# Suyashagarw/StreamOptima

Measured on AMD Instinct MI355X. Metric: encoded Mpixels/sec at 1080p & 4K, 1/2/4/8 GPUs; PSNR delta vs reference, higher is better.
Workload: dtype u8

## Files before the change

### include/streamoptima.h

```cpp
#ifndef STREAMOPTIMA_H
#define STREAMOPTIMA_H

#include <stddef.h>
#include <stdint.h>

#ifdef __cplusplus
extern "C" {
#endif

#define SO_OK 0
#define SO_E_INVALID (-1)
#define SO_E_UNSUPPORTED (-2)
#define SO_MAX_REF 4
#define SO_ABI_VERSION 1

int so_abi_version(void);
const char* so_last_error(void);

int so_me_full_search(const uint8_t* cur, const uint8_t* const* refs, int nref, int H,
                      int W, int bs, int sr, int32_t* out_best, int32_t* out_sub,
                      void* stream);

int so_inter_tq_recon(const uint8_t* cur, const uint8_t* const* refs, int nref, int H,
                      int W, int bs, const int32_t* best, const int32_t* sub, int qp_rd,
                      const int32_t* qp_row, int vbs, double lam, uint8_t* out_split,
                      int16_t* out_mv, int16_t* out_qtc, int32_t* out_tokens,
                      int32_t* out_mae_num, uint8_t* out_recon, int32_t* out_sse, void* stream);

size_t so_p_frame_scratch_elems(int H, int W, int bs, int vbs);

int so_encode_p_frame(const uint8_t* cur, const uint8_t* const* refs, int nref, int H,
                      int W, int bs, int sr, int qp_rd, const int32_t* qp_row, int vbs,
                      double lam, uint8_t* out_split, int16_t* out_mv, int16_t* out_qtc,
                      int32_t* out_tokens, int32_t* out_mae_num, uint8_t* out_recon,
                      int32_t* out_sse, int32_t* scratch, void* stream);

int so_encode_p_rows(const uint8_t* cur, const uint8_t* const* refs, int nref, int H, int W,
                     int bs, int sr, int by0, int by1, int qp_rd, const int32_t* qp_row,
                     int vbs, double lam, uint8_t* out_split, int16_t* out_mv,
                     int16_t* out_qtc, int32_t* out_tokens, int32_t* out_mae_num,
                     uint8_t* out_recon, int32_t* out_sse, int32_t* scratch, void* stream);

#define SO_OPT_RUN_2PASS_FUSED 1
#define SO_OPT_FASTME_SERIAL 2
#define SO_OPT_FASTME_SEGMENT 3
#define SO_OPT_FASTME_WARMUP 4
#define SO_OPT_COUNT_SAD_OPS 5
#define SO_OPT_TEST_LOSE_FLAG 6
#define SO_OPT_RUN_ZERO_SKIP 7
int so_set_option(int option, int value);
int so_get_option(int option);

#define SO_P_RUN_TIMEOUT_WORD 32
#define SO_P_RUN_FALLBACK_WORD 64
#define SO_P_RUN_SAD_OPS_WORD 66
#define SO_P_RUN_STALE_WORD 33
#define SO_P_RUN_GAP_WORD 34
#define SO_P_RUN_DIAG_WORD 96
#define SO_P_RUN_DIAG_MAGIC 0x534F0001u
size_t so_p_run_workspace_elems(int H, int W);
int so_p_run_resident_workgroups(int vbs);
int so_p_run_mode_resident_workgroups(int mode, int vbs);
int so_encode_p_run(const uint8_t* const* curs, int nframes, const uint8_t* ref0, int H, int W,
                    int bs, int sr, int qp_rd, const int32_t* qp_row, int vbs, double lam,
                    uint8_t* const* out_split,
                    int16_t* const* out_mv, int16_t* const* out_qtc, int32_t* const* out_tokens,
                    int32_t* const* out_mae_num, uint8_t* const* out_recon, int32_t* const* out_sse,
                    uint32_t* workspace, void* stream);

int so_p_run_2pass_fused(int H, int W);

int so_encode_p_run_2pass(const uint8_t* const* curs, int nframes, const uint8_t* ref0, int H, int W,
                          int bs, int sr, int qp_rd, const int32_t* qp_row, const int32_t* roi,
                          int qp_lo, int qp_hi, uint8_t* const* out_split, int16_t* const* out_mv,
                          int16_t* const* out_qtc, int32_t* const* out_tokens,
                          int32_t* const* out_mae_num, uint8_t* const* out_recon,
                          int32_t* const* out_sse, int32_t* const* out_qp_map, uint32_t* workspace,
                          void* stream);

int so_encode_p_runs(const uint8_t* const* curs, int nframes, const uint8_t* const* refs,
                     const int32_t* ref_frame, int H, int W, int bs, int sr, int qp_rd,
                     const int32_t* qp_row, int vbs, double lam, uint8_t* const* out_split,
                     int16_t* const* out_mv,
                     int16_t* const* out_qtc, int32_t* const* out_tokens, int32_t* const* out_mae_num,
                     uint8_t* const* out_recon, int32_t* const* out_sse, uint32_t* workspace,
                     void* stream);

int so_encode_p_run_stripe(const uint8_t* const* curs, int nframes, const uint8_t* ref0, int H, int W,
                           int bs, int sr, int by0, int by1, int qp_rd, const int32_t* qp_row,
                           uint8_t* const* out_split, int16_t* const* out_mv, int16_t* const* out_qtc,
                           int32_t* const* out_tokens, int32_t* const* out_mae_num,
                           uint8_t* const* out_recon, int32_t* const* out_sse, uint32_t* workspace,
                           int gbase, uint8_t* peer_up0, uint8_t* peer_dn0, long long stride,
                           const uint32_t* my_up_flags, const uint32_t* my_dn_flags,
                           uint32_t* peer_up_flags, uint32_t* peer_dn_flags, uint32_t epoch, int max_wg,
                           void* stream);

int so_stripe_halo_push(const uint8_t* plane, int H, int W, int by0, int by1, int gf, uint8_t* peer_up,
                        uint8_t* peer_dn, uint32_t* peer_up_flags, uint32_t* peer_dn_flags,
                        uint32_t epoch, void* stream);

int so_encode_p_run_fpipe2(const uint8_t* const* curs, int nframes, int H, int W, int bs, int sr,
                           int qp_rd, const int32_t* qp_row, int vbs, double lam,
                           uint8_t* const* out_split,
                           int16_t* const* out_mv, int16_t* const* out_qtc, int32_t* const* out_tokens,
                           int32_t* const* out_mae_num, uint8_t* const* out_recon,
                           int32_t* const* out_sse, uint32_t* workspace, const uint8_t* land0,
                           const uint32_t* land_flags, int slot0, uint8_t* peer_land0,
                           uint32_t* peer_flags, uint8_t* peer2_land0, uint32_t* peer2_flags,
                           const int32_t* push_to, int nslots, long long stride, uint32_t epoch,
                           int max_wg, void* stream);
int so_encode_p_run_fpipe_2pass(const uint8_t* const* curs, int nframes, int H, int W, int bs, int sr,
                                int qp_rd, const int32_t* qp_row, const int32_t* roi, int qp_lo,
                                int qp_hi, uint8_t* const* out_split, int16_t* const* out_mv,
                                int16_t* const* out_qtc, int32_t* const* out_tokens,
                                int32_t* const* out_mae_num, uint8_t* const* out_recon,
                                int32_t* const* out_sse, int32_t* const* out_qp_map, uint32_t* workspace,
                                const uint8_t* land0, const uint32_t* land_flags, int slot0,
                                uint8_t* peer_land0, uint32_t* peer_flags, uint8_t* peer2_land0,
                                uint32_t* peer2_flags, const int32_t* push_to, int nslots, long long stride,
                                uint32_t epoch, int max_wg, int p2lag, void* stream);
int so_frame_push(const uint8_t* plane, int H, int W, uint8_t* peer_plane, uint32_t* peer_flags,
                  uint32_t epoch, void* stream);

#define SO_IPC_HANDLE_BYTES 64
int so_alloc_uncached(size_t bytes, void** out);
int so_free_device(void* p);
int so_ipc_export(void* p, uint8_t* out_handle);
int so_ipc_open(const uint8_t* handle, void** out);
int so_ipc_close(void* p);
int so_copy_d2d(void* dst, const void* src, size_t bytes, void* stream);
int so_memset_d8(void* dst, int value, size_t bytes, void* stream);

size_t so_i_frame_scratch_elems(int H, int W, int bs);

int so_encode_i_frame(const uint8_t* cur, int H, int W, int bs, int sr, int qp_rd,
                      const int32_t* qp_row, int vbs, double lam, uint8_t* out_split,
                      int16_t* out_mv, int16_t* out_qtc, int32_t* out_tokens,
                      int32_t* out_mae_num, uint8_t* out_recon, int32_t* out_sse,
                      int32_t* scratch, void* stream);

int so_encode_i_rows(const uint8_t* cur, int H, int W, int bs, int sr, int by0, int by1,
                     int qp_rd, const int32_t* qp_row, int vbs, double lam, uint8_t* out_split,
                     int16_t* out_mv, int16_t* out_qtc, int32_t* out_tokens,
                     int32_t* out_mae_num, uint8_t* out_recon, int32_t* out_sse,
// ... 79 lines not shown
```

### streamoptima_amd/_lib.py

```python
from __future__ import annotations

import ctypes
import os
import threading

import torch

from .build import LIB_PATH

_lock = threading.Lock()
_lib = None

SO_OK = 0
SO_E_INVALID = -1
SO_E_UNSUPPORTED = -2
MAX_REF = 4

_vp = ctypes.c_void_p
_i = ctypes.c_int
_d = ctypes.c_double
_sz = ctypes.c_size_t

_SIGS = {
    "so_abi_version": ([], _i),
    "so_last_error": ([], ctypes.c_char_p),
    "so_me_full_search": ([_vp, _vp, _i, _i, _i, _i, _i, _vp, _vp, _vp], _i),
    "so_inter_tq_recon": ([_vp, _vp, _i, _i, _i, _i, _vp, _vp, _i, _vp, _i, _d, _vp, _vp, _vp, _vp,
                           _vp, _vp, _vp, _vp], _i),
    "so_p_frame_scratch_elems": ([_i, _i, _i, _i], _sz),
    "so_encode_p_frame": ([_vp, _vp, _i, _i, _i, _i, _i, _i, _vp, _i, _d, _vp, _vp, _vp, _vp, _vp,
                           _vp, _vp, _vp, _vp], _i),
    "so_encode_p_rows": ([_vp, _vp, _i, _i, _i, _i, _i, _i, _i, _i, _vp, _i, _d, _vp, _vp, _vp, _vp,
                          _vp, _vp, _vp, _vp, _vp], _i),
    "so_p_run_workspace_elems": ([_i, _i], _sz),
    "so_p_run_resident_workgroups": ([_i], _i),
    "so_p_run_mode_resident_workgroups": ([_i, _i], _i),
    "so_p_run_2pass_fused": ([_i, _i], _i),
    "so_encode_p_run": ([_vp, _i, _vp, _i, _i, _i, _i, _i, _vp, _i, _d, _vp, _vp, _vp, _vp, _vp, _vp, _vp, _vp, _vp],
                        _i),
    "so_encode_p_run_2pass": ([_vp, _i, _vp, _i, _i, _i, _i, _i, _vp, _vp, _i, _i, _vp, _vp, _vp, _vp, _vp, _vp, _vp,
                               _vp, _vp, _vp], _i),
    "so_encode_p_runs": ([_vp, _i, _vp, _vp, _i, _i, _i, _i, _i, _vp, _i, _d, _vp, _vp, _vp, _vp, _vp, _vp, _vp, _vp,
                          _vp], _i),
    "so_i_frame_scratch_elems": ([_i, _i, _i], _sz),
    "so_encode_i_frame": ([_vp, _i, _i, _i, _i, _i, _vp, _i, _d, _vp, _vp, _vp, _vp, _vp, _vp, _vp,
                           _vp, _vp], _i),
    "so_encode_i_rows": ([_vp, _i, _i, _i, _i, _i, _i, _i, _vp, _i, _d, _vp, _vp, _vp, _vp, _vp, _vp,
                          _vp, _vp, _vp], _i),
    "so_inter_recon": ([_vp, _i, _i, _i, _i, _i, _vp, _vp, _vp, _vp, _vp, _vp], _i),
    "so_intra_recon": ([_i, _i, _i, _i, _vp, _vp, _vp, _vp, _vp, _vp, _vp], _i),
    "so_sse_u8": ([_vp, _vp, ctypes.c_int64, _vp, _vp], _i),
    "so_block_xform": ([_vp, _i, _i, _i, _i, _vp, _vp, _vp, _vp], _i),
    "so_encode_p_run_stripe": ([_vp, _i, _vp, _i, _i, _i, _i, _i, _i, _i, _vp, _vp, _vp, _vp, _vp, _vp, _vp, _vp, _vp,
                                _i, _vp, _vp, ctypes.c_longlong, _vp, _vp, _vp, _vp, ctypes.c_uint32, _i, _vp], _i),
    "so_stripe_halo_push": ([_vp, _i, _i, _i, _i, _i, _vp, _vp, _vp, _vp, ctypes.c_uint32, _vp], _i),
    "so_alloc_uncached": ([_sz, ctypes.POINTER(ctypes.c_void_p)], _i),
    "so_free_device": ([_vp], _i),
    "so_ipc_export": ([_vp, _vp], _i),
    "so_ipc_open": ([_vp, ctypes.POINTER(ctypes.c_void_p)], _i),
    "so_ipc_close": ([_vp], _i),
    "so_copy_d2d": ([_vp, _vp, _sz, _vp], _i),
    "so_memset_d8": ([_vp, _i, _sz, _vp], _i),
    "so_pack_bound": ([_i, _i], _sz),
    "so_sum_i32_rows": ([_vp, _i, _i, _vp, _vp], _i),
    "so_unpack_frames": ([_i, _vp, _vp, _vp, _i, _i, _vp, _vp, _vp, _vp, _vp], _i),
    "so_encode_p_run_fpipe2": ([_vp, _i, _i, _i, _i, _i, _i, _vp, _i, _d,
                                _vp, _vp, _vp, _vp, _vp, _vp, _vp, _vp,
                                _vp, _vp, _i, _vp, _vp, _vp, _vp, _vp, _i,
                                ctypes.c_longlong, ctypes.c_uint32, _i, _vp], _i),
    "so_encode_p_run_fpipe_2pass": ([_vp, _i, _i, _i, _i, _i, _i, _vp, _vp, _i, _i,
                                     _vp, _vp, _vp, _vp, _vp, _vp, _vp, _vp, _vp,
                                     _vp, _vp, _i, _vp, _vp, _vp, _vp, _vp, _i,
                                     ctypes.c_longlong, ctypes.c_uint32, _i, _i, _vp], _i),
    "so_frame_push": ([_vp, _i, _i, _vp, _vp, ctypes.c_uint32, _vp], _i),
    "so_pack_frames": ([_i, _vp, _vp, _vp, _vp, _i, _i, _vp, _vp, ctypes.c_ulonglong, _vp], _i),
    "so_pack_frames_ex": ([_i, _vp, _vp, _vp, _vp, _i, _i, _vp, _vp, ctypes.c_ulonglong, _vp, _vp], _i),
    "so_fme_plane_stride": ([_i, _i], _sz),
    "so_fme_workspace_bytes": ([_i, _i, _i], _sz),
    "so_fme_planes": ([_vp, _i, _i, _i, _vp, _vp], _i),
    "so_me_search_ex": ([_vp, _vp, _i, _i, _i, _i, _i, _i, _i, _i, _vp, _vp, _vp, _vp], _i),
    "so_encode_p_rows_ex": ([_vp, _vp, _i, _i, _i, _i, _i, _i, _i, _i, _vp, _vp, _i, _d, _i, _i, _i, _vp, _i,
                             _vp, _vp, _vp, _vp, _vp, _vp, _vp, _vp, _vp], _i),
    "so_inter_recon_ex": ([_vp, _i, _i, _i, _i, _i, _vp, _vp, _i, _i, _vp, _vp, _vp, _vp, _vp, _vp], _i),
    "so_encode_i_rows_ex": ([_vp, _i, _i, _i, _i, _i, _i, _i, _vp, _vp, _i, _d, _vp, _vp, _vp, _vp, _vp, _vp,
                             _vp, _vp, _vp], _i),
    "so_intra_recon_ex": ([_i, _i, _i, _i, _vp, _vp, _vp, _vp, _vp, _vp, _vp, _vp], _i),
    "so_qp_map": ([_vp, _i, _i, _i, _i, _i, _i, _vp, _vp, _i, _i, _vp, _vp], _i),
    "so_set_option": ([_i, _i], _i),
    "so_get_option": ([_i], _i),
}

ME_FULL, ME_FAST, ME_FAST_PAR = 0, 1, 2
REUSE_ME = 1
TOKENS_ONLY = 2
OPT_RUN_2PASS_FUSED, OPT_FASTME_SERIAL, OPT_FASTME_SEGMENT, OPT_FASTME_WARMUP, OPT_COUNT_SAD_OPS = 1, 2, 3, 4, 5
OPT_RUN_ZERO_SKIP = 7
OPT_TEST_LOSE_FLAG = 6

EXPORTED = tuple(_SIGS)


class HipPathError(RuntimeError):
    """Raised when the gfx950 library is unavailable or a kernel call fails."""


def load(path: str | None = None):
    global _lib
    with _lock:
        if _lib is not None:
            return _lib
        p = path or os.environ.get("SO_LIB_PATH") or LIB_PATH
        if not os.path.exists(p):
            raise HipPathError(
                f"{p} is missing: build it with `python -m streamoptima_amd.build` (hipcc, gfx950). "
                "There is no CPU fallback for the encode path.")
        lib = ctypes.CDLL(p)
        for name, (args, res) in _SIGS.items():
            if p != LIB_PATH and not hasattr(lib, name):
                continue
            fn = getattr(lib, name)
            fn.argtypes = args
            fn.restype = res
        if lib.so_abi_version() != 1:
            raise HipPathError("libstreamoptima_hip.so ABI mismatch")
        _lib = lib
        return lib


def check(rc: int, what: str) -> None:
    if rc != SO_OK:
        msg = load().so_last_error().decode(errors="replace")
        if rc == SO_E_INVALID:
            raise ValueError(f"{what}: {msg}")
        if rc == SO_E_UNSUPPORTED:
            raise NotImplementedError(f"{what}: {msg}")
        raise HipPathError(f"{what}: HIP error {rc}: {msg}")


def set_option(opt: int, value: int) -> int:
    lib = load()
    old = lib.so_get_option(opt)
    check(lib.so_set_option(opt, int(value)), "so_set_option")
    return old


class option:

    def __init__(self, opt: int, value: int):
        self.opt, self.value, self.old = opt, value, None

    def __enter__(self):
        self.old = set_option(self.opt, self.value)
        return self

    def __exit__(self, *exc):
        set_option(self.opt, self.old)
        return False


def ptr(t) -> int | None:
    return None if t is None else t.data_ptr()


def ref_array(refs) -> ctypes.Array:
    arr = (ctypes.c_void_p * len(refs))(*[r.data_ptr() for r in refs])
    return arr


def stream_handle(device=None) -> int:
    return torch.cuda.current_stream(device).cuda_stream
```

### streamoptima_amd/csrc/so_block.h

```cpp
#pragma once
#include "so_common.h"
#include "so_dct.h"

namespace so {

SO_DEV void wave_sync() {
    __builtin_amdgcn_fence(__ATOMIC_RELEASE, "wavefront");
    __builtin_amdgcn_wave_barrier();
    __builtin_amdgcn_fence(__ATOMIC_ACQUIRE, "wavefront");
}

SO_DEV int scan_index(int n, int i, int j) {
    const int k = i + j;
    const int before = (k < n) ? (k * (k + 1)) / 2 : n * n - ((2 * n - 1 - k) * (2 * n - k)) / 2;
    const int first_i = (k < n) ? 0 : k - n + 1;
    return before + (i - first_i);
}

template <int G>
SO_DEV int group_sum(int v) {
#pragma unroll
    for (int m = G / 2; m >= 1; m >>= 1) v += __shfl_xor(v, m, 64);
    return v;
}
// ... 54 lines not shown
    const uint8_t* p = f + (size_t)y * W + x;
    if constexpr (NB == 16) {
        uint4 v = *reinterpret_cast<const uint4*>(p);
        uint32_t w[4] = {v.x, v.y, v.z, v.w};
#pragma unroll
        for (int k = 0; k < 16; ++k) out[k] = (w[k >> 2] >> (8 * (k & 3))) & 255;
    } else {
        uint2 v = *reinterpret_cast<const uint2*>(p);
        uint32_t w[2] = {v.x, v.y};
#pragma unroll
        for (int k = 0; k < 8; ++k) out[k] = (w[k >> 2] >> (8 * (k & 3))) & 255;
    }
}

template <int NB>
SO_DEV void store_row_u8(uint8_t* __restrict__ f, int W, int x, int y, const int* v) {
    uint32_t w[NB / 4];
#pragma unroll
    for (int k = 0; k < NB / 4; ++k)
        w[k] = (uint32_t)(v[4 * k] & 255) | ((uint32_t)(v[4 * k + 1] & 255) << 8) |
               ((uint32_t)(v[4 * k + 2] & 255) << 16) | ((uint32_t)(v[4 * k + 3] & 255) << 24);
    uint8_t* p = f + (size_t)y * W + x;
    if constexpr (NB == 16) *reinterpret_cast<uint4*>(p) = make_uint4(w[0], w[1], w[2], w[3]);
    else *reinterpret_cast<uint2*>(p) = make_uint2(w[0], w[1]);
}

template <int NB>
SO_DEV void store_row_i16(int16_t* __restrict__ p, const int* v) {
    uint32_t w[NB / 2];
#pragma unroll
    for (int k = 0; k < NB / 2; ++k) w[k] = (uint32_t)(uint16_t)v[2 * k] | ((uint32_t)(uint16_t)v[2 * k + 1] << 16);
    if constexpr (NB == 16) {
        reinterpret_cast<uint4*>(p)[0] = make_uint4(w[0], w[1], w[2], w[3]);
        reinterpret_cast<uint4*>(p)[1] = make_uint4(w[4], w[5], w[6], w[7]);
    } else {
        reinterpret_cast<uint4*>(p)[0] = make_uint4(w[0], w[1], w[2], w[3]);
    }
}

template <int NB>
SO_DEV void load_row_i16(const int16_t* __restrict__ p, int* v) {
    uint32_t w[NB / 2];
    if constexpr (NB == 16) {
        uint4 a = reinterpret_cast<const uint4*>(p)[0], b = reinterpret_cast<const uint4*>(p)[1];
        w[0] = a.x; w[1] = a.y; w[2] = a.z; w[3] = a.w; w[4] = b.x; w[5] = b.y; w[6] = b.z; w[7] = b.w;
    } else {
        uint4 a = reinterpret_cast<const uint4*>(p)[0];
        w[0] = a.x; w[1] = a.y; w[2] = a.z; w[3] = a.w;
    }
#pragma unroll
    for (int k = 0; k < NB / 2; ++k) {
        v[2 * k] = (int)(int16_t)(w[k] & 0xFFFF);
        v[2 * k + 1] = (int)(int16_t)(w[k] >> 16);
    }
}

template <int N, bool INVERSE, class T, class TWt = typename dct::Rfft<N>::TW>
SO_DEV void xform2d_rows(double* lds, int l, const T* in_row, double* out_row, const TWt& tw = TWt{}) {
    constexpr int P = N + 1;
    double v[N];
    if constexpr (N == 16 && __is_same(T, int)) {
        int* const li = reinterpret_cast<int*>(lds);
#pragma unroll
        for (int c = 0; c < N; ++c) li[l * P + c] = in_row[c];
        wave_sync();
        int x[N];
#pragma unroll
        for (int r = 0; r < N; ++r) x[r] = li[r * P + l];
        wave_sync();
        if constexpr (INVERSE) dct::dct3_16_i(x, v, tw); else dct::dct2_16_i(x, v, tw);
    } else {
#pragma unroll
        for (int c = 0; c < N; ++c) lds[l * P + c] = (double)in_row[c];
        wave_sync();
#pragma unroll
        for (int r = 0; r < N; ++r) v[r] = lds[r * P + l];
        if constexpr (INVERSE) dct::dct3<N>(v, tw); else dct::dct2<N>(v, tw);
    }
#pragma unroll
    for (int r = 0; r < N; ++r) lds[r * P + l] = v[r];
    wave_sync();
#pragma unroll
    for (int c = 0; c < N; ++c) v[c] = lds[l * P + c];
    if constexpr (INVERSE) dct::dct3<N>(v, tw); else dct::dct2<N>(v, tw);
#pragma unroll
    for (int c = 0; c < N; ++c) out_row[c] = v[c];
    wave_sync();
}

template <class TWt>
SO_DEV void xform2d_fwd_i_half(double* lds, int l, const int* in_row, double* out_row, const TWt& tw) {
    constexpr int N = 16, PI = N + 1, P = 9;
    const int hl = l >> 3, cl = l & 7;
    double v[N];
    {
        int* const li = reinterpret_cast<int*>(lds);
#pragma unroll
        for (int c = 0; c < N; ++c) li[l * PI + c] = in_row[c];
        wave_sync();
        int x[N];
#pragma unroll
        for (int r = 0; r < N; ++r) x[r] = li[r * PI + l];
        wave_sync();
        dct::dct2_16_i(x, v, tw);
    }
#pragma unroll
    for (int h = 0; h < 2; ++h) {
        if (hl == h) {
#pragma unroll
            for (int r = 0; r < N; ++r) lds[r * P + cl] = v[r];
        }
        wave_sync();
#pragma unroll
        for (int c = 0; c < 8; ++c) out_row[8 * h + c] = lds[l * P + c];
        wave_sync();
    }
    dct::dct2<N>(out_row, tw);
}

template <bool INVERSE, class T>
SO_DEV void xform2d_rows_half(double* lds, int l, const T* in_row, double* out_row) {
    constexpr int N = 16, P = 9;
    const int hl = l >> 3, cl = l & 7;
    double v[N];
#pragma unroll
    for (int h = 0; h < 2; ++h) {
#pragma unroll
        for (int c = 0; c < 8; ++c) lds[l * P + c] = (double)in_row[8 * h + c];
        wave_sync();
        if (hl == h) {
#pragma unroll
            for (int r = 0; r < N; ++r) v[r] = lds[r * P + cl];
        }
        wave_sync();
    }
    if constexpr (INVERSE) dct::dct3<N>(v); else dct::dct2<N>(v);
#pragma unroll
    for (int h = 0; h < 2; ++h) {
        if (hl == h) {
#pragma unroll
            for (int r = 0; r < N; ++r) lds[r * P + cl] = v[r];
        }
        wave_sync();
#pragma unroll
        for (int c = 0; c < 8; ++c) out_row[8 * h + c] = lds[l * P + c];
        wave_sync();
    }
    if constexpr (INVERSE) dct::dct3<N>(out_row); else dct::dct2<N>(out_row);
}

template <bool INVERSE, class T, class TWt = dct::TW8>
SO_DEV void xform2d_sub(double* lds, int l, const T (&in)[2][8], double (&out)[2][8], const TWt& tw = TWt{}) {
    const int j = l >> 2, r0 = l & 3;
    double* s = lds + j * 72;
    if constexpr (__is_same(T, int)) {
        int* const si = reinterpret_cast<int*>(s);
#pragma unroll
        for (int h = 0; h < 2; ++h)
#pragma unroll
            for (int c = 0; c < 8; ++c) si[(r0 + 4 * h) * 9 + c] = in[h][c];
        wave_sync();
        int x[2][8];
#pragma unroll
        for (int h = 0; h < 2; ++h)
#pragma unroll
            for (int r = 0; r < 8; ++r) x[h][r] = si[r * 9 + r0 + 4 * h];
// ... 179 lines not shown
```

### streamoptima_amd/csrc/so_capi.hip

```cpp
#include <stdarg.h>
#include <stdio.h>
#include <stdlib.h>
#include <string.h>

#include <atomic>
#include <vector>

#include <hip/hip_ext.h>

#include "so_common.h"
#include "so_run.h"

namespace so {

static thread_local char g_err[512] = "";

void set_error(const char* fmt, ...) {
    va_list ap;
    va_start(ap, fmt);
    vsnprintf(g_err, sizeof(g_err), fmt, ap);
    va_end(ap);
}

static std::atomic<int> g_opt[8] = {0, 1, 0, 32, 32, 0, 0, 0};

int option(int id) {
    return (id > 0 && id < 8) ? g_opt[id].load(std::memory_order_relaxed) : 0;
}

int me_launch(const uint8_t* cur, const RefSet& refs, int nref, int H, int W, int bs, int sr, int by0, int by1,
              int32_t* out_best, int32_t* out_sub, hipStream_t st);
int me_generic_launch(const uint8_t* cur, const RefSet& refs, const uint8_t* planes, size_t pstride, int nref, int H,
                      int W, int bs, int sr, int by0, int by1, int32_t* out_best, int32_t* out_sub, hipStream_t st);
int me_fme_launch(const uint8_t* cur, const uint8_t* planes, size_t pstride, int nref, int H, int W, int by0, int by1,
                  int32_t* out_best, int32_t* out_sub, hipStream_t st);
int fme_planes_launch(const uint8_t* ref, int H, int W, int wrap, uint8_t* out, size_t pstride, hipStream_t st);
int me_fastpred_launch(const uint8_t* cur, const uint8_t* const* ptrs, int nptr, int nref, int H, int W, int bs,
                       int fme, int by0, int by1, int serial, int32_t* out_best, int32_t* out_sub, int32_t* seg_ws,
                       hipStream_t st);
constexpr size_t kFastSegWords = 2 * 4096 * 6;
int p_tile_launch(const uint8_t* cur, const RefSet& refs, int H, int W, int by0, int by1, int qp_rd,
                  const int32_t* qp_row, const int32_t* qp_map, int32_t* out_best, uint8_t* out_split,
                  int16_t* out_mv, int16_t* out_qtc, int32_t* out_tokens, int32_t* out_mae, uint8_t* out_recon,
                  int32_t* out_sse, hipStream_t st, bool tokens_only = false, const int16_t* prev_mv = nullptr);

struct PackFrame {
    const uint8_t* split;
    const int16_t* mv;
    const int16_t* qtc;
    uint32_t* offs;
    uint8_t* out;
    int frame_type;
};
size_t pack_block_bound(int bs);
struct UnpackFrame {
    const uint8_t* in;
    const uint32_t* offs;
    uint8_t* split;
    int16_t* mv;
    int16_t* qtc;
    int frame_type;
};
int unpack_frames_launch(const UnpackFrame* frames, int nframes, int nb, int bs, int32_t* err, hipStream_t st);
int pack_frames_launch(const PackFrame* frames, int nframes, int nb, int bs, unsigned long long cap, uint32_t* totals,
                       hipStream_t st);
int stripe_halo_push_launch(const uint8_t* plane, int W, int by0, int by1, uint8_t* up, uint8_t* dn,
                            uint32_t* up_flags, uint32_t* dn_flags, int gf, uint32_t epoch, hipStream_t st);
int frame_push_launch(const uint8_t* plane, int H, int W, uint8_t* dst, uint32_t* flags, uint32_t epoch,
                      hipStream_t st);

#ifdef SO_AB
extern "C" int so_debug_ab_build(void) { return 1; }
#endif

static bool use_fused(int bs, int sr, int vbs, int nref) {
    if (bs != 16 || sr != 16 || vbs || nref != 1) return false;
#ifdef SO_AB
    const char* f = getenv("SO_FUSED");
    if (f && strcmp(f, "0") == 0) return false;
    const char* impl = getenv("SO_ME_IMPL");
    return impl == nullptr || impl[0] == 0;
#else
    return true;
#endif
}

int inter_tq_launch(const uint8_t* cur, const RefSet& refs, const uint8_t* planes, size_t pstride, int H, int W,
                    int bs, int by0, int by1, const int32_t* best, const int32_t* sub, int qp_rd, const int32_t* qp_row,
                    const int32_t* qp_map, int vbs, double lam, uint8_t* out_split, int16_t* out_mv, int16_t* out_qtc, int32_t* out_tokens,
                    int32_t* out_mae, uint8_t* out_recon, int32_t* out_sse, hipStream_t st);
int inter_tq_2pass_launch(const uint8_t* cur, const RefSet& refs, int H, int W, const int32_t* best, const int32_t* t1,
                          int qp_rd, const int32_t* qp_row, const int32_t* roi, int qp_lo, int qp_hi,
                          int32_t* out_qpmap, uint8_t* out_split, int16_t* out_mv, int16_t* out_qtc,
                          int32_t* out_tokens, int32_t* out_mae, uint8_t* out_recon, int32_t* out_sse,
                          hipStream_t st);
int inter_recon_launch(const RefSet& refs, const uint8_t* planes, size_t pstride, int H, int W, int bs, int qp,
                       const int32_t* qp_row, const int32_t* qp_map, const uint8_t* split, const int16_t* mv, const int16_t* qtc,
                       uint8_t* out_recon, hipStream_t st);
int intra_encode_launch(const uint8_t* cur, int H, int W, int bs, int sr, int by0, int by1, int qp_rd,
                        const int32_t* qp_row, const int32_t* qp_map, int vbs, double lam, uint8_t* out_split, int16_t* out_mv,
                        int16_t* out_qtc, int32_t* out_tokens, int32_t* out_mae, uint8_t* out_recon,
                        int32_t* out_sse, uint8_t* idres, hipStream_t st);
int intra_recon_launch(int H, int W, int bs, int sr, int qp, const int32_t* qp_row, const int32_t* qp_map,
                       const uint8_t* split,
                       const int16_t* mv, const int16_t* qtc, uint8_t* out_recon, uint8_t* idres,
                       hipStream_t st);

static int check_vbs(const char* fn, int vbs, double lam) {
    if (vbs != 0 && vbs != 1) {
        set_error("%s: vbs must be 0 or 1", fn);
// ... 110 lines not shown
    for (int m = 32; m >= 1; m >>= 1) acc += __shfl_xor(acc, m, 64);
    if ((threadIdx.x & 63) == 0) part[threadIdx.x >> 6] = acc;
    __syncthreads();
    if (threadIdx.x == 0) {
        long long t = 0;
#pragma unroll
        for (int w = 0; w < kSumThreads / 64; ++w) t += part[w];
        out[blockIdx.x] = t;
    }
}

__global__ void __launch_bounds__(256) sse_kernel(const uint8_t* __restrict__ a, const uint8_t* __restrict__ b,
                                                  int64_t n, unsigned long long* __restrict__ out) {
    __shared__ unsigned long long part[4];
    unsigned long long acc = 0;
    const int64_t n16 = n / 16;
    const int64_t stride = (int64_t)gridDim.x * blockDim.x;
    for (int64_t i = (int64_t)blockIdx.x * blockDim.x + threadIdx.x; i < n16; i += stride) {
        const uint4 va = reinterpret_cast<const uint4*>(a)[i];
        const uint4 vb = reinterpret_cast<const uint4*>(b)[i];
        const uint32_t wa[4] = {va.x, va.y, va.z, va.w}, wb[4] = {vb.x, vb.y, vb.z, vb.w};
        uint32_t s = 0;
#pragma unroll
        for (int k = 0; k < 4; ++k)
#pragma unroll
            for (int e = 0; e < 4; ++e) {
                const int d = (int)((wa[k] >> (8 * e)) & 255) - (int)((wb[k] >> (8 * e)) & 255);
                s += (uint32_t)(d * d);
            }
        acc += s;
    }
    if (blockIdx.x == 0 && threadIdx.x == 0)
        for (int64_t i = n16 * 16; i < n; ++i) {
            const int d = (int)a[i] - (int)b[i];
            acc += (unsigned long long)(d * d);
        }
#pragma unroll
    for (int m = 32; m >= 1; m >>= 1) acc += __shfl_xor(acc, m, 64);
    if ((threadIdx.x & 63) == 0) part[threadIdx.x >> 6] = acc;
    __syncthreads();
    if (threadIdx.x == 0) atomicAdd(out, part[0] + part[1] + part[2] + part[3]);
}

__global__ void __launch_bounds__(256)
qp_map_kernel(const int32_t* __restrict__ tokens, int nbx, int by0, int qp_rd, const int32_t* __restrict__ qp_row,
              const int32_t* __restrict__ roi, int qp_lo, int qp_hi, int32_t* __restrict__ out) {
    __shared__ long long part[4];
    const int by = by0 + blockIdx.x;
    const int32_t* t = tokens ? tokens + (size_t)blockIdx.x * nbx : nullptr;
    long long m = 0;
    if (t) {
        for (int bx = threadIdx.x; bx < nbx; bx += blockDim.x) m += t[bx];
#pragma unroll
        for (int s = 32; s >= 1; s >>= 1) m += __shfl_xor(m, s, 64);
        if ((threadIdx.x & 63) == 0) part[threadIdx.x >> 6] = m;
        __syncthreads();
        m = part[0] + part[1] + part[2] + part[3];
    }
    const int base = qp_row ? qp_row[by] : qp_rd;
    for (int bx = threadIdx.x; bx < nbx; bx += blockDim.x) {
        int d = 0;
        if (t) {
            const long long tn = (long long)t[bx] * nbx;
            d = (tn >= 2 * m) + (tn >= 4 * m) - (2 * tn < m) - (4 * tn < m);
        }
        int q = base + d + (roi ? roi[(size_t)by * nbx + bx] : 0);
        q = q < qp_lo ? qp_lo : (q > qp_hi ? qp_hi : q);
        out[(size_t)by * nbx + bx] = q;
    }
}

}

using namespace so;

extern "C" {

int so_abi_version(void) { return SO_ABI_VERSION; }

int so_set_option(int opt, int value) {
    const bool ok = (opt == SO_OPT_RUN_2PASS_FUSED || opt == SO_OPT_FASTME_SERIAL || opt == SO_OPT_COUNT_SAD_OPS ||
                     opt == SO_OPT_RUN_ZERO_SKIP)
                        ? (value == 0 || value == 1)
                    : opt == SO_OPT_FASTME_SEGMENT                               ? value >= 1
                    : opt == SO_OPT_FASTME_WARMUP || opt == SO_OPT_TEST_LOSE_FLAG ? value >= 0
                                                                                 : false;
    if (!ok) {
        set_error("so_set_option: option %d value %d is unknown or out of range", opt, value);
        return SO_E_INVALID;
    }
    g_opt[opt].store(value, std::memory_order_relaxed);
    return SO_OK;
}

int so_get_option(int opt) { return option(opt); }

const char* so_last_error(void) { return g_err; }

int so_me_full_search(const uint8_t* cur, const uint8_t* const* refs, int nref, int H, int W, int bs,
                      int sr, int32_t* out_best, int32_t* out_sub, void* stream) {
    const char* fn = "so_me_full_search";
    SO_TRY(check_geom(fn, H, W, bs, out_sub != nullptr));
    SO_TRY(check_sr(fn, sr));
    SO_NEED(cur, fn);
    SO_NEED(out_best, fn);
    RefSet rs;
    SO_TRY(make_refs(fn, refs, nref, &rs));
    return me_launch(cur, rs, nref, H, W, bs, sr, 0, H / bs, out_best, out_sub, (hipStream_t)stream);
}

int so_inter_tq_recon(const uint8_t* cur, const uint8_t* const* refs, int nref, int H, int W, int bs,
                      const int32_t* best, const int32_t* sub, int qp_rd, const int32_t* qp_row, int vbs,
                      double lam, uint8_t* out_split, int16_t* out_mv, int16_t* out_qtc, int32_t* out_tokens,
                      int32_t* out_mae_num, uint8_t* out_recon, int32_t* out_sse, void* stream) {
    const char* fn = "so_inter_tq_recon";
    SO_TRY(check_geom(fn, H, W, bs, vbs));
    SO_TRY(check_qp(fn, qp_rd));
    SO_NEED(cur, fn); SO_NEED(best, fn); SO_NEED(out_split, fn); SO_NEED(out_mv, fn);
    SO_NEED(out_qtc, fn); SO_NEED(out_tokens, fn); SO_NEED(out_mae_num, fn); SO_NEED(out_recon, fn);
    if (vbs) SO_NEED(sub, fn);
    RefSet rs;
    SO_TRY(make_refs(fn, refs, nref, &rs));
    for (int i = 0; i < nref; ++i)
        if (refs[i] == out_recon) {
            set_error("%s: out_recon aliases refs[%d]", fn, i);
            return SO_E_INVALID;
        }
    return inter_tq_launch(cur, rs, nullptr, 0, H, W, bs, 0, H / bs, best, vbs ? sub : nullptr, qp_rd, qp_row, nullptr, vbs, lam,
                           out_split, out_mv, out_qtc, out_tokens, out_mae_num, out_recon, out_sse,
                           (hipStream_t)stream);
}

size_t so_p_frame_scratch_elems(int H, int W, int bs, int vbs) {
    if (bs <= 0) return 0;
    const size_t nb = (size_t)(W / bs) * (size_t)(H / bs);
    return nb * 4 + (vbs ? nb * 16 : 0) + kFastSegWords;
}

int so_encode_p_rows(const uint8_t* cur, const uint8_t* const* refs, int nref, int H, int W, int bs, int sr,
                     int by0, int by1, int qp_rd, const int32_t* qp_row, int vbs, double lam, uint8_t* out_split,
                     int16_t* out_mv, int16_t* out_qtc, int32_t* out_tokens, int32_t* out_mae_num,
                     uint8_t* out_recon, int32_t* out_sse, int32_t* scratch, void* stream) {
    const char* fn = "so_encode_p_rows";
    SO_TRY(check_geom(fn, H, W, bs, vbs));
    SO_TRY(check_sr(fn, sr));
    SO_TRY(check_qp(fn, qp_rd));
    SO_TRY(check_rows(fn, H, bs, by0, by1));
    SO_NEED(cur, fn); SO_NEED(scratch, fn); SO_NEED(out_split, fn); SO_NEED(out_mv, fn);
    SO_NEED(out_qtc, fn); SO_NEED(out_tokens, fn); SO_NEED(out_mae_num, fn); SO_NEED(out_recon, fn);
    RefSet rs;
    SO_TRY(make_refs(fn, refs, nref, &rs));
    for (int i = 0; i < nref; ++i)
        if (refs[i] == out_recon) {
            set_error("%s: out_recon aliases refs[%d]", fn, i);
            return SO_E_INVALID;
        }
    const size_t nbs = (size_t)(W / bs) * (size_t)(by1 - by0);
    int32_t* best = scratch;
    int32_t* sub = vbs ? scratch + nbs * 4 : nullptr;
    hipStream_t st = (hipStream_t)stream;
    if (use_fused(bs, sr, vbs, nref))
        return p_tile_launch(cur, rs, H, W, by0, by1, qp_rd, qp_row, nullptr, best, out_split, out_mv, out_qtc,
                             out_tokens, out_mae_num, out_recon, out_sse, st);
    SO_TRY(me_launch(cur, rs, nref, H, W, bs, sr, by0, by1, best, sub, st));
    return inter_tq_launch(cur, rs, nullptr, 0, H, W, bs, by0, by1, best, sub, qp_rd, qp_row, nullptr, vbs, lam, out_split,
                           out_mv, out_qtc, out_tokens, out_mae_num, out_recon, out_sse, st);
}

int so_encode_p_frame(const uint8_t* cur, const uint8_t* const* refs, int nref, int H, int W, int bs, int sr,
                      int qp_rd, const int32_t* qp_row, int vbs, double lam, uint8_t* out_split,
                      int16_t* out_mv, int16_t* out_qtc, int32_t* out_tokens, int32_t* out_mae_num,
                      uint8_t* out_recon, int32_t* out_sse, int32_t* scratch, void* stream) {
    if (bs <= 0) {
        set_error("so_encode_p_frame: block_size %d", bs);
        return SO_E_UNSUPPORTED;
    }
    return so_encode_p_rows(cur, refs, nref, H, W, bs, sr, 0, H / bs, qp_rd, qp_row, vbs, lam, out_split, out_mv,
                            out_qtc, out_tokens, out_mae_num, out_recon, out_sse, scratch, stream);
}

size_t so_p_run_workspace_elems(int H, int W) {
    if (H <= 0 || W <= 0) return 0;
    return p_run_workspace_words(H, W);
}

int so_p_run_resident_workgroups(int vbs) {
    const int n = p_run_capacity(vbs ? 1 : 0);
    if (n <= 0) {
        set_error("so_p_run_resident_workgroups: device query failed");
        return SO_E_INVALID;
    }
    return n;
}

int so_p_run_2pass_fused(int H, int W) {
    return H > 0 && W > 0 && option(SO_OPT_RUN_2PASS_FUSED) == 1 && p_run_2pass_fused_ok(H, W) ? 1 : 0;
}

int so_p_run_mode_resident_workgroups(int mode, int vbs) {
    if (mode < 0 || mode > 4 || (vbs && mode != 0 && mode != 2)) {
        set_error("so_p_run_mode_resident_workgroups: mode %d%s", mode, vbs ? " with vbs (modes 0, 2)" : " (0..4)");
        return SO_E_INVALID;
    }
    const int n = p_run_capacity(vbs ? 1 : 0, mode);
    if (n <= 0) {
        set_error("so_p_run_mode_resident_workgroups: device query failed");
        return SO_E_INVALID;
    }
    return n;
}

int so_encode_p_run(const uint8_t* const* curs, int nframes, const uint8_t* ref0, int H, int W, int bs, int sr,
                    int qp_rd, const int32_t* qp_row, int vbs, double lam, uint8_t* const* out_split,
                    int16_t* const* out_mv, int16_t* const* out_qtc, int32_t* const* out_tokens,
                    int32_t* const* out_mae_num, uint8_t* const* out_recon, int32_t* const* out_sse,
                    uint32_t* workspace, void* stream) {
    const char* fn = "so_encode_p_run";
    SO_TRY(check_geom(fn, H, W, bs, vbs));
    SO_TRY(check_vbs(fn, vbs, lam));
    SO_TRY(check_sr(fn, sr));
    SO_TRY(check_qp(fn, qp_rd));
    if (bs != 16 || sr != 16 || W % 128 != 0) {
        set_error("%s: covers bs 16 / sr 16 / W %% 128 == 0 (call so_encode_p_frame per frame)", fn);
        return SO_E_UNSUPPORTED;
    }
    if (nframes <= 0) return SO_OK;
    SO_NEED(curs, fn); SO_NEED(ref0, fn); SO_NEED(out_split, fn); SO_NEED(out_mv, fn); SO_NEED(out_qtc, fn);
    SO_NEED(out_tokens, fn); SO_NEED(out_mae_num, fn); SO_NEED(out_recon, fn); SO_NEED(workspace, fn);
    std::vector<PFrameOut> outs((size_t)nframes);
    for (int i = 0; i < nframes; ++i) {
        SO_NEED(curs[i], fn); SO_NEED(out_split[i], fn); SO_NEED(out_mv[i], fn); SO_NEED(out_qtc[i], fn);
        SO_NEED(out_tokens[i], fn); SO_NEED(out_mae_num[i], fn); SO_NEED(out_recon[i], fn);
        for (int j = -1; j < i; ++j)
            if (out_recon[i] == (j < 0 ? ref0 : out_recon[j])) {
                set_error("%s: out_recon[%d] aliases ref0 or another frame's reconstruction", fn, i);
                return SO_E_INVALID;
            }
        outs[i] = PFrameOut{out_split[i], out_mv[i], out_qtc[i], out_tokens[i], out_mae_num[i], out_recon[i],
                            out_sse ? out_sse[i] : nullptr};
    }
    return p_run_launch(curs, nframes, ref0, H, W, qp_rd, qp_row, vbs, lam, outs.data(), workspace,
                        (hipStream_t)stream);
}

int so_encode_p_runs(const uint8_t* const* curs, int nframes, const uint8_t* const* refs, const int32_t* ref_frame,
                     int H, int W, int bs, int sr, int qp_rd, const int32_t* qp_row, int vbs, double lam,
                     uint8_t* const* out_split, int16_t* const* out_mv, int16_t* const* out_qtc,
                     int32_t* const* out_tokens, int32_t* const* out_mae_num, uint8_t* const* out_recon,
                     int32_t* const* out_sse, uint32_t* workspace, void* stream) {
    const char* fn = "so_encode_p_runs";
    SO_TRY(check_geom(fn, H, W, bs, vbs));
    SO_TRY(check_vbs(fn, vbs, lam));
    SO_TRY(check_sr(fn, sr));
    SO_TRY(check_qp(fn, qp_rd));
    if (bs != 16 || sr != 16 || W % 128 != 0) {
        set_error("%s: covers bs 16 / sr 16 / W %% 128 == 0 (call so_encode_p_frame per frame)", fn);
        return SO_E_UNSUPPORTED;
    }
    if (nframes <= 0) return SO_OK;
    SO_NEED(curs, fn); SO_NEED(refs, fn); SO_NEED(ref_frame, fn); SO_NEED(out_split, fn); SO_NEED(out_mv, fn);
    SO_NEED(out_qtc, fn); SO_NEED(out_tokens, fn); SO_NEED(out_mae_num, fn); SO_NEED(out_recon, fn);
    SO_NEED(workspace, fn);
    std::vector<PFrameOut> outs((size_t)nframes);
    std::vector<int> deps((size_t)nframes);
    int conc = 0;
    for (int i = 0; i < nframes; ++i) {
        SO_NEED(curs[i], fn); SO_NEED(out_split[i], fn); SO_NEED(out_mv[i], fn); SO_NEED(out_qtc[i], fn);
        SO_NEED(out_tokens[i], fn); SO_NEED(out_mae_num[i], fn); SO_NEED(out_recon[i], fn);
        const int d = ref_frame[i];
        if (d >= i || d < -1) {
            set_error("%s: ref_frame[%d] = %d (must be -1 or an earlier frame of the list)", fn, i, d);
            return SO_E_INVALID;
// ... 679 lines not shown
```

### streamoptima_amd/csrc/so_me.hip

```cpp
#include <stdlib.h>
#include <string.h>

#include <cstring>
#include <map>
#include <mutex>
#include <utility>

#include "so_block.h"
#include "so_common.h"
#include "so_dpp.h"
#include "so_run.h"

namespace so {

SO_DEV uint64_t me_key(uint32_t sad, uint32_t l1, uint32_t ref, uint32_t scan) {
    return ((uint64_t)sad << 32) | ((uint64_t)l1 << 24) | ((uint64_t)ref << 16) | (uint64_t)scan;
}
constexpr uint64_t kNoKey = ~0ull;
constexpr uint32_t kDenseSadOps = 1152u * 256u;
#define SO_OPS_ADD(p, v) do { if (L.count_ops) atomicAdd((p), (v)); } while (0)

SO_DEV void decode_key(uint64_t k, int sr, int32_t* out) {
    if (k == kNoKey) {
        out[0] = 0; out[1] = 0; out[2] = 0; out[3] = -1;
        return;
    }
    const int d = 2 * sr + 1;
    const int scan = (int)(k & 0xFFFF);
    out[0] = scan / d - sr;
    out[1] = scan % d - sr;
    out[2] = (int)((k >> 16) & 0xFF);
    out[3] = (int)(k >> 32);
}

template <int BS, bool SUB>
struct MeWGeo {
    static constexpr int SR = 16, D = 33, NT = 17;
    static constexpr int TBX = 128 / BS;
    static constexpr int TPY = SUB ? 32 : 64;
    static constexpr int TBY = TPY / BS;
    static constexpr int TPX = 128;
    static constexpr int WR = TPY + 2 * SR;
    static constexpr int RPD = (TPX + 2 * SR) / 4 + 1;
    static constexpr int CSTRIDE = WR * RPD + 8;
    static constexpr int NBLK = TBX * TBY;
    static constexpr int NW = SUB ? 8 : 16, NTHREADS = NW * 64;
};

typedef const __attribute__((address_space(4))) uint32_t* const_u32p;
typedef const volatile __attribute__((address_space(3))) uint32_t* lds_vu32p;

template <int NR, int NDW>
SO_DEV void load_cur_sgpr(const uint8_t* __restrict__ cur, int W, int x, int y, uint32_t (&cr)[NR][NDW]) {
#pragma unroll
    for (int r = 0; r < NR; ++r) {
        const_u32p p = (const_u32p)(cur + (size_t)(y + r) * W + x);
#pragma unroll
        for (int k = 0; k < NDW; ++k) cr[r][k] = p[k];
    }
}


template <int WR, int RPD, int CS, int NT>
SO_DEV void stage_window(uint32_t* win, const uint8_t* __restrict__ ref, int H, int W, int gx0, int gy0, int tid) {
    constexpr int N = WR * RPD, IT = (N + NT - 1) / NT;
    uint32_t a[IT], b[IT];
#pragma unroll
    for (int k = 0; k < IT; ++k) {
        const int i = tid + k * NT;
        const int wr = i / RPD, m = i - wr * RPD;
        const int gy = gy0 + wr, gx = gx0 + 4 * m;
        a[k] = 0;
        b[k] = 0;
        if (i < N && gy >= 0 && gy < H) {
            const uint8_t* rp = ref + (size_t)gy * W;
            if (gx >= 0 && gx + 4 <= W) a[k] = *reinterpret_cast<const uint32_t*>(rp + gx);
            if (gx + 4 >= 0 && gx + 8 <= W) b[k] = *reinterpret_cast<const uint32_t*>(rp + gx + 4);
        }
    }
#pragma unroll
    for (int k = 0; k < IT; ++k) {
        const int i = tid + k * NT;
        if (i < N) {
            uint32_t* d = win + i;
            d[0] = a[k];
            d[CS] = __builtin_amdgcn_alignbyte(b[k], a[k], 1);
            d[2 * CS] = __builtin_amdgcn_alignbyte(b[k], a[k], 2);
            d[3 * CS] = __builtin_amdgcn_alignbyte(b[k], a[k], 3);
// ... 329 lines not shown
        else decode_key(keys[i], 2 * SR, out_sub + (b * 4 + ((i - G::NBLK) & 3)) * 4);
    }
}

__global__ void __launch_bounds__(256)
fme_planes_kernel(const uint8_t* __restrict__ ref, int H, int W, int wrap, uint8_t* __restrict__ out, size_t pstride) {
    const int q = blockIdx.x * blockDim.x + threadIdx.x;
    const int qpr = W >> 2;
    if (q >= qpr * H) return;
    const int i = q / qpr, j0 = (q - i * qpr) * 4;
    const uint8_t* r0 = ref + (size_t)i * W + j0;
    const bool down = i + 1 < H;
    const uint8_t* r1 = down ? r0 + W : r0;
    uint32_t p00 = 0, p01 = 0, p10 = 0, p11 = 0;
    const uint32_t w0 = *reinterpret_cast<const uint32_t*>(r0), w1 = *reinterpret_cast<const uint32_t*>(r1);
    const bool right = j0 + 4 < W;
    const int e0 = right ? r0[4] : 0, e1 = right ? r1[4] : 0;
#pragma unroll
    for (int k = 0; k < 4; ++k) {
        const int a = (w0 >> (8 * k)) & 255, c = (w1 >> (8 * k)) & 255;
        const bool rk = j0 + k + 1 < W;
        const int a2 = k < 3 ? (int)((w0 >> (8 * k + 8)) & 255) : e0;
        const int c2 = k < 3 ? (int)((w1 >> (8 * k + 8)) & 255) : e1;
        int h0 = a + a2, h1 = c + c2;
        if (wrap) { h0 &= 255; h1 &= 255; }
        p00 |= (uint32_t)a << (8 * k);
        if (rk) p01 |= (uint32_t)((h0 + 1) >> 1) << (8 * k);
        if (down) p10 |= (uint32_t)((a + c + 1) >> 1) << (8 * k);
        if (down && rk) p11 |= (uint32_t)((h0 + h1 + 3) >> 2) << (8 * k);
    }
    const size_t o = (size_t)i * W + j0;
    *reinterpret_cast<uint32_t*>(out + o) = p00;
    *reinterpret_cast<uint32_t*>(out + pstride + o) = p01;
    *reinterpret_cast<uint32_t*>(out + 2 * pstride + o) = p10;
    *reinterpret_cast<uint32_t*>(out + 3 * pstride + o) = p11;
}

int fme_planes_launch(const uint8_t* ref, int H, int W, int wrap, uint8_t* out, size_t pstride, hipStream_t st) {
    const int n = (W / 4) * H;
    hipLaunchKernelGGL(fme_planes_kernel, dim3((n + 255) / 256), dim3(256), 0, st, ref, H, W, wrap, out, pstride);
    return check_launch("fme_planes_kernel");
}

int me_fme_launch(const uint8_t* cur, const uint8_t* planes, size_t pstride, int nref, int H, int W, int by0, int by1,
                  int32_t* out_best, int32_t* out_sub, hipStream_t st) {
    const int nbx = W / 16, nrows = by1 - by0;
    if (nrows <= 0) return SO_OK;
    const bool sub = out_sub != nullptr;
    const int tby = (sub ? MeWGeo<16, true>::TPY : MeWGeo<16, false>::TPY) / 16;
    const dim3 grid(((nbx + 7) / 8) * ((nrows + tby - 1) / tby));
    if (sub)
        hipLaunchKernelGGL((me_fme_kernel<true>), grid, dim3(MeWGeo<16, true>::NTHREADS), 0, st, cur, planes, pstride,
                           nref, H, W, by0, by1, out_best, out_sub);
    else
        hipLaunchKernelGGL((me_fme_kernel<false>), grid, dim3(MeWGeo<16, false>::NTHREADS), 0, st, cur, planes,
                           pstride, nref, H, W, by0, by1, out_best, out_sub);
    return check_launch("me_fme_kernel");
}

#ifndef SO_SEA2_WPE
#define SO_SEA2_WPE 6
#endif
#ifndef SO_SEA_CAP
#define SO_SEA_CAP 384
#endif
#ifndef SO_SEA_CAP_VBS
#define SO_SEA_CAP_VBS 384
#endif
#ifndef SO_DENSE_THR
#define SO_DENSE_THR 8
#endif
#ifndef SO_DENSE_PROBE
#define SO_DENSE_PROBE 16
#endif
#ifndef SO_VBS_HALVES
#define SO_VBS_HALVES 0
#endif
#ifndef SO_B4_PD
#define SO_B4_PD 2
#endif
#ifndef SO_PTILE_WPE16
#define SO_PTILE_WPE16 8
#endif
template <int NW_, int TPX_ = 128>
struct Sea2GeoT {
    static constexpr int SR = 16, NT = 17;
    static constexpr int TPX = TPX_, TBX = TPX / 16, TPY = 32, TBY = 2;
    static constexpr int WR = TPY + 2 * SR;
    static constexpr int WD = (TPX + 2 * SR) / 4;
    static constexpr int RP = WD + 1;
    static constexpr int B4R = WR - 3, B4C = TPX + 2 * SR - 3, B4P = 4 * RP;
    static constexpr int TQ_BPW = TPX == 128 ? 4 : 2;
    static constexpr int B4BAND = NW_ >= 16 ? 3 : 6;
    static constexpr int B4NB = (B4R + B4BAND - 1) / B4BAND;
    static constexpr int B4RS = B4NB * B4BAND;
    static constexpr int NBLK = TBX * TBY;
    static constexpr int NW = NW_, NTHREADS = NW * 64;
    static constexpr int CAP = SO_SEA_CAP, CAPV = SO_SEA_CAP_VBS;
    static constexpr int CAPLV = SO_VBS_HALVES ? 2 * CAPV : CAPV;
    static constexpr int CAPL = CAP > CAPLV ? CAP : CAPLV;
    static constexpr int DCS = WR * RP + 8;
    static constexpr int CPD = TPX / 4 + 1;
    static_assert(WD * B4NB <= NTHREADS, "byte-sum threads");
};
using Sea2Geo = Sea2GeoT<8>;

template <int RP>
SO_DEV uint32_t win_u32(const uint32_t* win, int row, int col) {
    lds_vu32p p = (lds_vu32p)(win + row * RP + (col >> 2));
    return __builtin_amdgcn_alignbyte(p[1], p[0], (uint32_t)(col & 3));
}

#ifdef SO_STAMPS
__device__ unsigned long long* g_sea_stamps = nullptr;
__device__ unsigned long long* g_run_stamps = nullptr;
__shared__ unsigned long long* s_stamp_rec;
#define SO_SEA_STAMP(i, v) do { if (tid == 0 && s_stamp_rec) s_stamp_rec[(i)] = (v); } while (0)
#define SO_STAMP_REC_SET(p) do { if (threadIdx.x == 0) s_stamp_rec = (p); } while (0)
extern "C" int so_debug_set_sea_stamps(void* p) {
    return (int)hipMemcpyToSymbol(HIP_SYMBOL(g_sea_stamps), &p, sizeof(p));
}
extern "C" int so_debug_set_run_stamps(void* p) {
    return (int)hipMemcpyToSymbol(HIP_SYMBOL(g_run_stamps), &p, sizeof(p));
}
#else
#define SO_STAMP_REC_SET(p) do { } while (0)
#define SO_SEA_STAMP(i, v) do { } while (0)
#endif

#define SO_MARK_NAMES(X) X(loop_top) X(stage_cur) X(stage_cur_int) X(stage_cur_edge) X(cur_sums) X(wait) \
    X(poll_iter) X(stage_win) X(stage_win_int) X(stage_win_edge) X(dense_tile) X(dense_tile_block) X(byte_sums) \
    X(block_top) X(bound) X(umin) X(umin_edge) X(ballots) X(bal_row) X(dense_fallback) X(survivors) X(sur_one) X(sur_le4) X(sur_pass) \
    X(search_end) X(decode_keys) X(tq_residual) X(tq_fwd) X(tq_quant) X(tq_tokens) X(tq_qtc_store) X(tq_inv) \
    X(tq_recon) X(tq_sse_records) X(post) X(done_flag) X(task_end) X(vbs_block) X(vbs_umin) X(vbs_list_a) \
    X(vbs_pass) X(vbs_list_b) X(vbs_final) X(vbs_dense) X(vbs_fwd) X(vbs_fwd_sub) X(vbs_final_q) X(vbs_inv) \
    X(vbs_inv_split) X(vbs_inv_end) X(wait_w0) X(keys_tail) X(p1_tq) X(p1_flag) X(p2_wait) X(p2_sums) X(p2_tq) \
    X(p2_flag)
#define SO_MARK_ENUM(n) kMark_##n,
enum SoMarkId { SO_MARK_NAMES(SO_MARK_ENUM) kMarkCount };
#undef SO_MARK_ENUM
#if defined(SO_MARKS_COUNT)
__device__ unsigned* g_mark_counts = nullptr;
__shared__ unsigned s_mark_cnt[64];
extern "C" int so_debug_set_mark_counts(void* p) {
    return (int)hipMemcpyToSymbol(HIP_SYMBOL(g_mark_counts), &p, sizeof(p));
}
SO_DEV void so_mark_hit(int id) {
    uint64_t sv, m;
    uint32_t f;
    asm volatile(
        "s_mov_b64 %0, exec\n\t"
        "s_ff1_i32_b64 %2, exec\n\t"
        "s_lshl_b64 %1, 1, %2\n\t"
        "s_and_b64 exec, exec, %1\n\t"
        "ds_add_u32 %3, %4\n\t"
        "s_mov_b64 exec, %0"
        : "=&s"(sv), "=&s"(m), "=&s"(f)
        : "v"((uint32_t)(uintptr_t)&s_mark_cnt[id]), "v"(1u)
        : "memory", "scc");
}
#define SO_MARK(name) so_mark_hit(kMark_##name)
#elif defined(SO_MARKS)
#define SO_MARK(name) asm volatile(";SO_MARK " #name)
#else
#define SO_MARK(name) do { } while (0)
#endif

SO_DEV int opaque_tid() {
    int t = threadIdx.x;
    asm volatile("" : "+v"(t));
    return t;
}

struct Sea2Lds {
    uint32_t* win;
    uint32_t* b4w;
// ... 326 lines not shown
        nB = vbs_list_from_masks<NT>(mylist, mB, cbase, 32 * 33 + d2, (uint32_t)CAP);
    } else {
#pragma unroll
        for (int t = 0; t <= NT; ++t) {
            const bool pass = t < NT ? (any_sub(T[t], Bt[t]) && ((amask >> t) & 1u) == 0u)
                                     : (ok2 && any_sub(l2T, l2B) && !(lb2 <= qU));
            const uint64_t bal = __builtin_amdgcn_ballot_w64(pass);
            if (bal) {
                const uint32_t pos = nB + lane_prefix(bal);
                if (pass && pos < (uint32_t)CAP) mylist[pos] = (uint16_t)(t < NT ? cbase + t : 32 * 33 + d2);
                nB += (uint32_t)__builtin_popcountll(bal);
            }
        }
    }
    if (nB > (uint32_t)CAP) return false;
    if (lane == 0) SO_OPS_ADD(&L.st[2], 16u * ((nB + 15) / 16) * 256u);
    __builtin_amdgcn_fence(__ATOMIC_RELEASE, "wavefront");
    __builtin_amdgcn_wave_barrier();
    __builtin_amdgcn_fence(__ATOMIC_ACQUIRE, "wavefront");
    vbs_eval_list<G>(L, mylist, nB, cs, bxl, byl, lane, bestB, best0, best1);
    SO_MARK(vbs_final);
    const uint64_t kb = wave_min_u64_dpp(bestB);
    const auto widen = [](uint32_t k) {
        return ((uint64_t)(k >> 17) << 32) | ((uint64_t)((k >> 11) & 63u) << 24) | (uint64_t)(k & 2047u);
    };
    const uint64_t kTL = widen(wave_min_u32(top ? best0 : ~0u)), kTR = widen(wave_min_u32(top ? best1 : ~0u));
    const uint64_t kBL = widen(wave_min_u32(top ? ~0u : best0)), kBR = widen(wave_min_u32(top ? ~0u : best1));
    if (lane == 0) {
        unsigned long long* const ks = L.keys;
        if (kb < ks[u]) ks[u] = kb;
        unsigned long long* const sk = ks + G::NBLK + 4 * u;
        if (kTL < sk[0]) sk[0] = kTL;
        if (kTR < sk[1]) sk[1] = kTR;
        if (kBL < sk[2]) sk[2] = kBL;
        if (kBR < sk[3]) sk[3] = kBR;
    }
    return true;
}

template <class G, class Pre = NoPre, bool VBS = false, int LISTS = 0>
SO_DEV void sea2_tile(const Sea2Lds& L, int tile, const uint8_t* __restrict__ cur, const RefSet& refs, int nref,
                      int H, int W, int by0, int by1, int probe, const Pre& pre = Pre(),
                      const int* dense_flag = nullptr, const int16_t* prev_mv = nullptr) {
    constexpr int SR = G::SR, TBX = G::TBX, TBY = G::TBY, RP = G::RP, NT = G::NT;
    constexpr int B4P = G::B4P, CAP = G::CAP, CP = G::TPX;
#ifdef SO_NO_MV_HINT
    prev_mv = nullptr;
#endif
    uint32_t* const win = L.win;
    uint32_t* const b4w = L.b4w;
    uint8_t* const b4 = reinterpret_cast<uint8_t*>(b4w);
    uint32_t* const curt = L.curt;
    uint32_t* const a4 = L.a4;
    uint16_t* const list = L.list;
    unsigned long long* const keys = L.keys;

    const int nbx = W / 16;
    const int tiles_x = (nbx + TBX - 1) / TBX;
    const int tx = tile % tiles_x, ty = tile / tiles_x;
    const bool ballot_lists = LISTS == 2 || (LISTS == 0 && SO_VBS_BALLOT_LATENCY && VBS &&
                                             tiles_x * ((H / 16 + TBY - 1) / TBY) < (int)gridDim.x);
    const int bx0 = tx * TBX, byt0 = by0 + ty * TBY;
    const int x0 = bx0 * 16, y0 = byt0 * 16;
    const int tid = opaque_tid();
    const int wave = __builtin_amdgcn_readfirstlane(tid >> 6);
    uint32_t& st_fb = L.st[0];
    if (tid == 0) st_fb = 0;
    uint32_t& st_ops = L.st[2];
    if (tid == 0) {
        uint32_t ops0 = L.count_ops ? G::NBLK * 16 * 4 * 4 : 0u;
        asm volatile("" : "+v"(ops0));
        st_ops = ops0;
    }
#ifdef SO_STAMPS
    uint32_t& st_sur = L.st[1];
    if (tid == 0) st_sur = 0;
    SO_SEA_STAMP(0, __builtin_amdgcn_s_memrealtime());
    SO_SEA_STAMP(1, __builtin_amdgcn_s_memtime());
#endif

    SO_MARK(stage_cur);
    for (int i = tid; i < G::NBLK * (VBS ? 5 : 1); i += G::NTHREADS) keys[i] = kNoKey;
    constexpr int WTPR = G::NTHREADS / G::WR, WNPT = (RP + WTPR - 1) / WTPR;
    static_assert(G::NTHREADS % G::WR == 0, "window staging");
    const int wwr = tid / WTPR, wc0 = tid - wwr * WTPR;
    const bool win_int = x0 - SR >= 0 && x0 - SR + 4 * RP <= W && y0 - SR >= 0 && y0 - SR + G::WR <= H;
    if (x0 + CP <= W && y0 + G::TPY <= H) {
        constexpr int TPR = G::NTHREADS / G::TPY, NPT = (CP / 4) / TPR;
        static_assert(G::NTHREADS % G::TPY == 0 && (CP / 4) % TPR == 0, "current-tile staging");
        SO_MARK(stage_cur_int);
        const int rr = tid / TPR, c0 = tid - rr * TPR;
        const uint32_t* src = reinterpret_cast<const uint32_t*>(cur + (size_t)(y0 + rr) * W + x0) + c0;
        uint32_t v[NPT];
#pragma unroll
        for (int k = 0; k < NPT; ++k) v[k] = src[k * TPR];
#pragma unroll
        for (int k = 0; k < NPT; ++k) curt[rr * G::CPD + c0 + k * TPR] = v[k];
    } else {
        SO_MARK(stage_cur_edge);
        constexpr int N = G::TPY * CP / 4, IT = (N + G::NTHREADS - 1) / G::NTHREADS;
        uint32_t v[IT];
#pragma unroll
        for (int k = 0; k < IT; ++k) {
            const int i = tid + k * G::NTHREADS;
            const int rr = i / (CP / 4), m = i - rr * (CP / 4);
            const int gy = y0 + rr, gx = x0 + 4 * m;
            v[k] = 0;
            if (i < N && gy < H && gx + 4 <= W) v[k] = *reinterpret_cast<const uint32_t*>(cur + (size_t)gy * W + gx);
        }
#pragma unroll
        for (int k = 0; k < IT; ++k)
            if (tid + k * G::NTHREADS < N) {
                const int i = tid + k * G::NTHREADS, rr = i / (CP / 4);
                curt[i + rr] = v[k];
            }
    }
    __syncthreads();
    SO_MARK(cur_sums);
    for (int i = tid; i < G::NBLK * 16; i += G::NTHREADS) {
        const int blk = i >> 4, j = (i >> 2) & 3, ii = i & 3;
        const int rr = (blk / TBX) * 16 + 4 * j, m = (blk % TBX) * 4 + ii;
        uint32_t sum = 0;
#pragma unroll
        for (int q = 0; q < 4; ++q) sum = __builtin_amdgcn_sad_u8(curt[(rr + q) * G::CPD + m], 0u, sum);
        reinterpret_cast<uint8_t*>(a4)[i] = (uint8_t)(sum >> 4);
    }
    uint32_t* const grab = L.lcount;
    const auto next_block = [&](int u) -> int {
#ifdef SO_SEA_STATIC
        return u + G::NW;
#else
        (void)u;
        uint32_t nx = 0;
        if ((tid & 63) == 0) nx = __hip_atomic_fetch_add(grab, 1u, __ATOMIC_RELAXED, __HIP_MEMORY_SCOPE_WORKGROUP);
        return (int)__builtin_amdgcn_readfirstlane(nx);
#endif
    };
    for (int r = 0; r < nref; ++r) {
        const uint8_t* ref = refs.p[r];
        SO_MARK(wait);
        if (r == 0) pre();
        SO_MARK(stage_win);
        if (tid == 0) *grab = (uint32_t)G::NW;
        __syncthreads();
        if (r == 0) SO_SEA_STAMP(2, __builtin_amdgcn_s_memtime());
        if (win_int) {
            SO_MARK(stage_win_int);
            uint32_t wv0[WNPT];
            const uint32_t* src = reinterpret_cast<const uint32_t*>(ref + (size_t)(y0 - SR + wwr) * W + (x0 - SR)) + wc0;
#pragma unroll
            for (int k = 0; k < WNPT; ++k)
                if (wc0 + k * WTPR < RP) wv0[k] = src[k * WTPR];
#pragma unroll
            for (int k = 0; k < WNPT; ++k)
                if (wc0 + k * WTPR < RP) win[wwr * RP + wc0 + k * WTPR] = wv0[k];
        } else {
            SO_MARK(stage_win_edge);
            constexpr int N = G::WR * RP, IT = (N + G::NTHREADS - 1) / G::NTHREADS;
            uint32_t v[IT];
#pragma unroll
            for (int k = 0; k < IT; ++k) {
                const int i = tid + k * G::NTHREADS;
                const int wr = i / RP, m = i - wr * RP;
                const int gy = y0 - SR + wr, gx = x0 - SR + 4 * m;
                v[k] = 0;
                if (i < N && gy >= 0 && gy < H && gx >= 0 && gx + 4 <= W)
                    v[k] = *reinterpret_cast<const uint32_t*>(ref + (size_t)gy * W + gx);
            }
#pragma unroll
            for (int k = 0; k < IT; ++k)
                if (tid + k * G::NTHREADS < N) win[tid + k * G::NTHREADS] = v[k];
        }
        __syncthreads();
        if (r == 0) SO_SEA_STAMP(3, __builtin_amdgcn_s_memtime());
        if (probe == 5) continue;
        if (dense_flag && __builtin_amdgcn_readfirstlane(*dense_flag)) {
            SO_MARK(dense_tile);
            const int c1 = L.dense4;
            if (c1 != 0) {
                uint32_t* const cp = win + c1;
                for (int i = tid; i < G::WR * RP; i += G::NTHREADS) {
                    const uint32_t a = win[i], b = win[i + 1];
                    cp[i] = __builtin_amdgcn_alignbyte(b, a, 1);
                    cp[G::DCS + i] = __builtin_amdgcn_alignbyte(b, a, 2);
                    cp[2 * G::DCS + i] = __builtin_amdgcn_alignbyte(b, a, 3);
                }
                __syncthreads();
            }
#pragma unroll 1
            for (int u = wave; u < G::NBLK; u = next_block(u)) {
                SO_MARK(dense_tile_block);
                const int bxl = u % TBX, byl = u / TBX;
                if (bx0 + bxl >= nbx || byt0 + byl >= by1) continue;
                const int x = x0 + bxl * 16, y = y0 + byl * 16;
                if (c1 != 0) {
                    if (VBS && x != 0 && y != 0)
                        wave_dense_block<16, true, RP, G::DCS>(win, keys, G::NBLK, cur, W, H, x, y, bxl, byl, u, tid, r,
                                                               FmePhase{0, 0}, c1);
                    else
                        wave_dense_block<16, false, RP, G::DCS>(win, keys, G::NBLK, cur, W, H, x, y, bxl, byl, u, tid,
                                                                r, FmePhase{0, 0}, c1);
                } else if (VBS && x != 0 && y != 0)
                    wave_dense_block<16, true, RP, 0, false, true>(win, keys, G::NBLK, cur, W, H, x, y, bxl, byl, u,
                                                                   tid, r);
                else
                    wave_dense_block<16, false, RP, 0, false, true>(win, keys, G::NBLK, cur, W, H, x, y, bxl, byl, u,
                                                                    tid, r);
                if ((tid & 63) == 0) {
                    atomicAdd(&st_fb, 1u);
                    SO_OPS_ADD(&st_ops, kDenseSadOps);
                }
            }
            continue;
        }
        SO_MARK(byte_sums);
        if (tid == 0) SO_OPS_ADD(&st_ops, (uint32_t)(G::WD * G::B4NB * (G::B4BAND + 3) * 4 * 4));
        if (tid < G::WD * G::B4NB) {
            const int m = tid % G::WD, band = tid / G::WD;
            const int r0 = band * G::B4BAND;
            constexpr int NR = G::B4BAND + 3;
            uint32_t h[NR][2];
            lds_vu32p p = (lds_vu32p)(win + r0 * RP + m);
#pragma unroll
            for (int i = 0; i < NR; ++i) {
                const uint32_t w0 = p[i * RP], w1 = p[i * RP + 1];
                h[i][0] = __builtin_amdgcn_sad_hi_u8(__builtin_amdgcn_alignbyte(w1, w0, 2), 0u,
                                                     __builtin_amdgcn_sad_u8(w0, 0u, 0u));
                h[i][1] = __builtin_amdgcn_sad_hi_u8(__builtin_amdgcn_alignbyte(w1, w0, 3), 0u,
                                                     __builtin_amdgcn_sad_u8(__builtin_amdgcn_alignbyte(w1, w0, 1), 0u, 0u));
            }
            typedef unsigned short so_v2u16 __attribute__((ext_vector_type(2)));
            uint8_t* const ob = b4 + r0 * B4P + m;
#pragma unroll
            for (int i = 0; i < G::B4BAND; ++i)
#pragma unroll
                for (int j = 0; j < 2; ++j) {
                    const uint32_t sum = h[i][j] + h[i + 1][j] + h[i + 2][j] + h[i + 3][j];
                    const uint32_t q = __builtin_bit_cast(uint32_t, __builtin_bit_cast(so_v2u16, sum) >> (so_v2u16){4, 4});
// ... 208 lines not shown
                for (int rr = 0; rr < 4; ++rr)
#pragma unroll
                    for (int k = 0; k < 4; ++k) cr[rr][k] = curt[crow0 + (4 * q + rr) * G::CPD + k];
#pragma unroll 1
                for (uint32_t s0 = 0; s0 < nsur; s0 += 16) {
                    SO_MARK(sur_pass);
                    const bool act = s0 + (uint32_t)sidx < nsur;
                    const int cand = act ? (int)mylist[s0 + sidx] : cs;
                    const int dxi = cand / 33, di = cand - dxi * 33;
                    const int col = bxl * 16 + dxi;
                    const uint32_t sh = (uint32_t)(col & 3);
                    int wo = (byl * 16 + di + 4 * q) * RP + (col >> 2);
                    asm volatile("" : "+v"(wo));
                    uint32_t sad = 0;
#pragma unroll
                    for (int rr = 0; rr < 4; ++rr) {
                        lds_vu32p p = (lds_vu32p)(win + wo + rr * RP);
                        const uint32_t q0 = p[0], q1 = p[1], q2 = p[2], q3 = p[3], q4 = p[4];
                        sad = __builtin_amdgcn_sad_u8(cr[rr][0], __builtin_amdgcn_alignbyte(q1, q0, sh), sad);
                        sad = __builtin_amdgcn_sad_u8(cr[rr][1], __builtin_amdgcn_alignbyte(q2, q1, sh), sad);
                        sad = __builtin_amdgcn_sad_u8(cr[rr][2], __builtin_amdgcn_alignbyte(q3, q2, sh), sad);
                        sad = __builtin_amdgcn_sad_u8(cr[rr][3], __builtin_amdgcn_alignbyte(q4, q3, sh), sad);
                    }
                    sad = quad_sum_u32(sad);
                    const int dx = dxi - 16, dy = di - 16;
                    const uint64_t key = me_key(sad, (uint32_t)((dx < 0 ? -dx : dx) + (dy < 0 ? -dy : dy)),
                                                (uint32_t)r, (uint32_t)cand);
                    best = (act && key < best) ? key : best;
                }
            }
            best = wave_min_u64_dpp(best);
            if (lane == 0 && best < keys[u]) keys[u] = best;
        }
    }
    SO_MARK(search_end);
    __syncthreads();
}

__global__ void __launch_bounds__(Sea2Geo::NTHREADS) __attribute__((amdgpu_waves_per_eu(SO_SEA2_WPE)))
me_sea2_kernel(const uint8_t* __restrict__ cur, RefSet refs, int nref, int H, int W, int by0, int by1,
               int32_t* __restrict__ out_best, int probe) {
    using G = Sea2Geo;
    constexpr int SR = G::SR, TBX = G::TBX, TBY = G::TBY, RP = G::RP, B4P = G::B4P;
    __shared__ uint32_t win[G::WR * RP + 4];
    __shared__ uint32_t b4w[(G::B4RS * B4P + 4) / 4];
    __shared__ uint32_t curt[G::TPY * G::CPD];
    __shared__ uint32_t a4[G::NBLK * 4];
    __shared__ uint16_t list[G::NW * G::CAPL];
    __shared__ uint32_t lcount[G::NW];
    __shared__ unsigned long long keys[G::NBLK];
    __shared__ uint32_t st[3];
    const Sea2Lds L{win, b4w, curt, a4, list, lcount, keys, st};
    SO_STAMP_REC_SET(g_sea_stamps ? g_sea_stamps + (size_t)blockIdx.x * 12 : nullptr);
    sea2_tile<Sea2Geo>(L, blockIdx.x, cur, refs, nref, H, W, by0, by1, probe);

    const int tid = threadIdx.x;
    const int nbx = W / 16;
    const int tiles_x = (nbx + TBX - 1) / TBX;
    const int bx0 = (blockIdx.x % tiles_x) * TBX, byt0 = by0 + (blockIdx.x / tiles_x) * TBY;
    SO_SEA_STAMP(5, __builtin_amdgcn_s_memtime());
    for (int i = tid; i < G::NBLK; i += G::NTHREADS) {
        const int gbx = bx0 + i % TBX, gby = byt0 + i / TBX;
        if (gbx >= nbx || gby >= by1) continue;
        decode_key(keys[i], SR, out_best + ((size_t)(gby - by0) * nbx + gbx) * 4);
    }
#ifdef SO_STAMPS
    if (tid == 0) {
        uint32_t hw, xcc;
        asm volatile("s_getreg_b32 %0, hwreg(HW_REG_HW_ID)" : "=s"(hw));
        asm volatile("s_getreg_b32 %0, hwreg(HW_REG_XCC_ID)" : "=s"(xcc));
        SO_SEA_STAMP(6, __builtin_amdgcn_s_memtime());
        SO_SEA_STAMP(7, __builtin_amdgcn_s_memrealtime());
        SO_SEA_STAMP(8, ((unsigned long long)xcc << 32) | hw);
        SO_SEA_STAMP(9, ((unsigned long long)st[0] << 32) | st[1]);
    }
#endif
}

constexpr int kTqScratch = 16 * 17;
#ifndef SO_PTILE_TOK_HALF
#define SO_PTILE_TOK_HALF 1
#endif
constexpr int kTqScratchHalf = 16 * 9;
#ifndef SO_FWD_MFMA
#define SO_FWD_MFMA 0
#endif
template <class G, bool HALFTQ = false>
struct PTileGeo {
    static constexpr int B4 = (G::B4RS * G::B4P + 4) / 4;
    static constexpr int LIST = G::NW * G::CAPL / 2;
    static constexpr int TQD = G::NBLK * (HALFTQ ? kTqScratchHalf : kTqScratch);
    static constexpr int U64 = ((B4 + LIST + 1) / 2 > TQD) ? (B4 + LIST + 1) / 2 : TQD;
};
constexpr int kTqScratchVbs = 288;
template <class G>
struct PTileGeoVbs {
    static constexpr int TQD = G::NBLK * kTqScratchVbs;
    static constexpr int U64 = ((PTileGeo<G>::B4 + PTileGeo<G>::LIST + 1) / 2 > TQD)
                                   ? (PTileGeo<G>::B4 + PTileGeo<G>::LIST + 1) / 2 : TQD;
};

template <int RP>
SO_DEV void win_row16(const uint32_t* win, int row, int col, uint32_t (&w)[4]) {
    lds_vu32p p = (lds_vu32p)(win + row * RP + (col >> 2));
    const uint32_t sh = (uint32_t)(col & 3);
    const uint32_t q0 = p[0], q1 = p[1], q2 = p[2], q3 = p[3], q4 = p[4];
    w[0] = __builtin_amdgcn_alignbyte(q1, q0, sh);
    w[1] = __builtin_amdgcn_alignbyte(q2, q1, sh);
    w[2] = __builtin_amdgcn_alignbyte(q3, q2, sh);
    w[3] = __builtin_amdgcn_alignbyte(q4, q3, sh);
}

typedef uint32_t so_v4u __attribute__((ext_vector_type(4)));

struct MeRec {
    uint16_t v[4];
    SO_DEV int operator[](int k) const { return k < 3 ? (int)(int16_t)v[k] : (v[3] == 0xFFFFu ? -1 : (int)v[3]); }
    SO_DEV void set(const int32_t (&r)[4]) {
#pragma unroll
        for (int k = 0; k < 4; ++k) v[k] = (uint16_t)r[k];
    }
};

template <class G, bool VBS = false, bool HALFTQ = false>
struct PTileLds {
    static constexpr int NU = G::NBLK * (VBS ? 5 : 1);
    uint32_t win[G::WR * G::RP + 4];
    uint32_t curt[G::TPY * G::CPD];
    uint32_t a4[G::NBLK * 4];
    uint32_t lcount[G::NW];
    unsigned long long keys[NU];
    uint32_t st[3];
    MeRec mer[NU];
    int32_t msum[G::TBY];
    uint32_t fwd_flags;
    alignas(16) double un[VBS ? PTileGeoVbs<G>::U64 : PTileGeo<G, HALFTQ>::U64];
    uint8_t vsp[VBS ? G::NBLK : 1];
};

struct PHalo {
    uint8_t* up;
    uint8_t* dn;
    int up_end, dn_begin;
};

#ifdef SO_TQ_TW_LITERAL
#define SO_TQ_TW() dct::TW16{}
#define SO_TQ_TW8() dct::TW8{}
#else
#define SO_TQ_TW() dct::tw16_table()
#define SO_TQ_TW8() dct::tw8_table()
#endif
template <class G, bool SC1, bool HALO = false, bool TOK = false, bool HALFTQ = false, bool ZSKIP = false>
SO_DEV void tq16_exact(PTileLds<G, false, HALFTQ>& S, int g, int l, double* scratch, int bx0, int byt0, int nbx, int by0, int by1,
                       int W, int qp_rd, const int32_t* __restrict__ qp_row, const int32_t* __restrict__ qp_map,
                       const PFrameOut& o, const PHalo& hl = PHalo{}, bool qs = false) {
    constexpr int SR = G::SR, TBX = G::TBX;
    const int bxl = g % TBX, byl = g / TBX;
    const int gbx = bx0 + bxl, gby = byt0 + byl;
    if (gbx < nbx && gby < by1) {
        const size_t b = (size_t)(gby - by0) * nbx + gbx;
        const int x = gbx * 16, y = gby * 16;
        const int qpr = qp_map ? qp_map[(size_t)gby * nbx + gbx] : (qp_row ? qp_row[gby] : qp_rd);
        const int dx = S.mer[g][0], dy = S.mer[g][1], rf = S.mer[g][2], sad = S.mer[g][3];
        const int prow = byl * 16 + SR + dy + l, pcol = bxl * 16 + SR + dx;
        const uint32_t* crow = S.curt + (byl * 16 + l) * G::CPD + bxl * 4;
        double* dl = scratch;
        constexpr double kRne = 0x1.8p52;
        int q[16];
        if (qs) {
            const so_v4u* qr = reinterpret_cast<const so_v4u*>(reinterpret_cast<const int16_t*>(dl) + l * 16);
#pragma unroll
            for (int h = 0; h < 2; ++h) {
                const so_v4u v = qr[h];
#pragma unroll
                for (int e = 0; e < 4; ++e) {
                    q[8 * h + 2 * e] = (int)(int16_t)(v[e] & 0xFFFFu);
                    q[8 * h + 2 * e + 1] = (int)v[e] >> 16;
                }
            }
        } else {
            SO_MARK(tq_residual);
            int res[16];
            {
                uint32_t pw[4];
                win_row16<G::RP>(S.win, prow, pcol, pw);
#pragma unroll
                for (int k = 0; k < 4; ++k) {
                    const uint32_t cw = crow[k];
#pragma unroll
                    for (int e = 0; e < 4; ++e)
                        res[4 * k + e] = (int)((cw >> (8 * e)) & 255) - (int)((pw[k] >> (8 * e)) & 255);
                }
            }
            double tcr[16];
            SO_MARK(tq_fwd);
            static_assert(!HALFTQ || TOK, "the half scratch carries the forward transform only");
            if constexpr (HALFTQ)
                xform2d_fwd_i_half(dl, l, res, tcr, SO_TQ_TW());
            else
                xform2d_rows<16, false>(dl, l, res, tcr, SO_TQ_TW());
            SO_MARK(tq_quant);
#pragma unroll
            for (int c = 0; c < 16; ++c)
                q[c] = (int)(uint32_t)__builtin_bit_cast(
                    uint64_t, __builtin_amdgcn_ldexp(__builtin_rint(tcr[c]), -q_exp_fast<16>(l, c, qpr)) + kRne);
        }
        SO_MARK(tq_tokens);
        const int tok = block_tokens<16>(nullptr, l, q);
        if constexpr (TOK) {
            if (l == 0) o.tokens[b] = tok;
            return;
        }
        SO_MARK(tq_qtc_store);
        store_row_i16<16>(o.qtc + b * 256 + l * 16, q);
        const auto finish = [&](const int (&rec)[16]) -> int {
            if constexpr (SC1) {
                so_v4u v;
#pragma unroll
                for (int k = 0; k < 4; ++k)
                    v[k] = (uint32_t)(rec[4 * k] & 255) | ((uint32_t)(rec[4 * k + 1] & 255) << 8) |
                           ((uint32_t)(rec[4 * k + 2] & 255) << 16) | ((uint32_t)(rec[4 * k + 3] & 255) << 24);
                uint8_t* rp = o.recon + (size_t)(y + l) * W + x;
                asm volatile("global_store_dwordx4 %0, %1, off sc1" ::"v"(rp), "v"(v) : "memory");
                if constexpr (HALO) {
                    if (hl.up && y + l < hl.up_end) {
                        uint8_t* q2 = hl.up + (size_t)(y + l) * W + x;
                        asm volatile("global_store_dwordx4 %0, %1, off sc0 sc1" ::"v"(q2), "v"(v) : "memory");
                    }
                    if (hl.dn && y + l >= hl.dn_begin) {
                        uint8_t* q2 = hl.dn + (size_t)(y + l) * W + x;
                        asm volatile("global_store_dwordx4 %0, %1, off sc0 sc1" ::"v"(q2), "v"(v) : "memory");
                    }
                }
            } else {
                store_row_u8<16>(o.recon, W, x, y + l, rec);
            }
            SO_MARK(tq_sse_records);
            int e2 = 0;
            if (o.sse) {
#pragma unroll
                for (int k = 0; k < 4; ++k) {
                    const uint32_t cw = crow[k];
#pragma unroll
                    for (int e = 0; e < 4; ++e) {
                        const int d = (int)((cw >> (8 * e)) & 255) - (rec[4 * k + e] & 255);
                        e2 += d * d;
                    }
                }
                e2 = group_sum<16>(e2);
            }
            return e2;
        };
        const auto full = [&]() -> int {
            int dq[16];
            double rd[16];
            dequant_row_int<16>(q, l, qpr, dq);
            SO_MARK(tq_inv);
            xform2d_rows<16, true>(dl, l, dq, rd, SO_TQ_TW());
            SO_MARK(tq_recon);
            int rec[16];
            {
                uint32_t pw[4];
                win_row16<G::RP>(S.win, prow, pcol, pw);
#pragma unroll
                for (int c = 0; c < 16; ++c)
                    rec[c] = (int)((pw[c >> 2] >> (8 * (c & 3))) & 255) +
                             (int)(uint32_t)__builtin_bit_cast(uint64_t, rd[c] + kRne);
            }
            return finish(rec);
        };
        int sse;
        if constexpr (ZSKIP) {
            if (__builtin_amdgcn_ballot_w64(tok != 1) == 0) {
                int rec[16];
                uint32_t pw[4];
                win_row16<G::RP>(S.win, prow, pcol, pw);
#pragma unroll
                for (int c = 0; c < 16; ++c) rec[c] = (int)((pw[c >> 2] >> (8 * (c & 3))) & 255);
                sse = finish(rec);
            } else {
                sse = full();
            }
        } else {
            sse = full();
        }
        if (l < 12) o.mv[b * 12 + l] = (int16_t)(l == 0 ? dx : l == 1 ? dy : l == 2 ? rf : 0);
        if (l == 0) {
            o.split[b] = 0;
            o.tokens[b] = tok;
            o.mae[b] = sad;
            if (o.sse) o.sse[b] = sse;
        }
    }
}

__constant__ float kDctCos32[17] = {
    0x1.6a09e6p-2f, 0x1.684b9cp-2f, 0x1.63150cp-2f, 0x1.5a730cp-2f, 0x1.4e7aeap-2f, 0x1.3f4a24p-2f,
    0x1.2d062ep-2f, 0x1.17dc14p-2f, 0x1.000000p-2f, 0x1.cb598cp-3f, 0x1.92469cp-3f, 0x1.5553e4p-3f,
    0x1.1517a8p-3f, 0x1.a4608ap-4f, 0x1.1a855ep-4f, 0x1.1be352p-5f, 0.0f};

SO_DEV float dct16_f32(int u, int r) {
    if (u == 0) return 0.25f;
    const int j = ((2 * r + 1) * u) & 63;
    const int m = j <= 32 ? j : 64 - j;
    return m <= 16 ? kDctCos32[m] : -kDctCos32[32 - m];
}

typedef float so_v4f __attribute__((ext_vector_type(4)));
constexpr float kFwdBound = 2.6e-7f;

template <class G>
SO_DEV void fwd_mfma(PTileLds<G>& S, int g, int ln, const float (&cs)[4], int bx0, int byt0, int nbx, int by1,
                     int qp_rd, const int32_t* __restrict__ qp_row, const int32_t* __restrict__ qp_map) {
    constexpr int SR = G::SR, TBX = G::TBX;
    const int bxl = g % TBX, byl = g / TBX;
    const int gbx = bx0 + bxl, gby = byt0 + byl;
    if (gbx >= nbx || gby >= by1) return;
    const int qpr = qp_map ? qp_map[(size_t)gby * nbx + gbx] : (qp_row ? qp_row[gby] : qp_rd);
    const int r = ln & 15, c4 = ln >> 4;
    const int dx = S.mer[g][0], dy = S.mer[g][1];
    const uint32_t cw = S.curt[(byl * 16 + r) * G::CPD + bxl * 4 + c4];
    const uint32_t pw = win_u32<G::RP>(S.win, byl * 16 + SR + dy + r, bxl * 16 + SR + dx + 4 * c4);
    float a[4];
    uint32_t sab = 0;
#pragma unroll
    for (int s = 0; s < 4; ++s) {
        const int d = (int)((cw >> (8 * s)) & 255) - (int)((pw >> (8 * s)) & 255);
        a[s] = (float)d;
        sab += (uint32_t)(d < 0 ? -d : d);
    }
    sab = wave_sum_u32(sab);
    so_v4f y = {0.f, 0.f, 0.f, 0.f}, z = {0.f, 0.f, 0.f, 0.f};
#pragma unroll
    for (int s = 0; s < 4; ++s) y = __builtin_amdgcn_mfma_f32_16x16x4f32(a[s], cs[s], y, 0, 0, 0);
#pragma unroll
    for (int s = 0; s < 4; ++s) z = __builtin_amdgcn_mfma_f32_16x16x4f32(cs[s], y[s], z, 0, 0, 0);
    const float delta = __builtin_fmaf((float)sab, kFwdBound, 0x1p-20f);
    bool near = qpr < 1;
    int16_t* qd = reinterpret_cast<int16_t*>(S.un + g * kTqScratch);
#pragma unroll
    for (int i = 0; i < 4; ++i) {
        const int u = 4 * c4 + i, k = q_exp_fast<16>(u, r, qpr);
        const float zi = z[i];
        const float mid = __builtin_amdgcn_ldexpf(__builtin_floorf(__builtin_amdgcn_ldexpf(zi, -k)) + 0.5f, k);
        near |= __builtin_fabsf(__builtin_fabsf(zi - mid) - 0.5f) <= delta;
        qd[u * 16 + r] = (int16_t)(int)__builtin_rintf(__builtin_amdgcn_ldexpf(__builtin_rintf(zi), -k));
    }
#ifdef SO_FWD_FORCE
    near = SO_FWD_FORCE;
#endif
    if (__builtin_amdgcn_ballot_w64(near) != 0 && ln == 0) atomicOr(&S.fwd_flags, 1u << g);
}

template <int NBLK>
SO_DEV int fwd_order(uint32_t m, int p) {
    const int nf = __builtin_popcount(m);
    uint32_t s = p < nf ? m : (~m & ((1u << NBLK) - 1u));
    for (int t = p < nf ? p : p - nf; t > 0; --t) s &= s - 1u;
    return __builtin_ctz(s);
}

template <int RP>
SO_DEV void win_row8(const uint32_t* win, int row, int col, uint32_t (&w)[2]) {
    lds_vu32p p = (lds_vu32p)(win + row * RP + (col >> 2));
    const uint32_t sh = (uint32_t)(col & 3);
    const uint32_t q0 = p[0], q1 = p[1], q2 = p[2];
    w[0] = __builtin_amdgcn_alignbyte(q1, q0, sh);
    w[1] = __builtin_amdgcn_alignbyte(q2, q1, sh);
}

template <bool SC1, bool HALO>
SO_DEV void store_rec_row(const PFrameOut& o, const PHalo& hl, int W, int x, int yy, const int* rec, int n) {
    uint8_t* rp = o.recon + (size_t)yy * W + x;
// ... 336 lines not shown
                       int by0, int by1, int qp_rd, const int32_t* __restrict__ qp_row,
                       const int32_t* __restrict__ qp_map, int32_t* __restrict__ out_best, const PFrameOut& o,
                       const Pre& pre = Pre(), const PHalo& hl = PHalo{}, double lam = 0.0,
                       const int* dense_flag = nullptr, int32_t* fb_out = nullptr, int count_ops = 0,
                       const Post& post = Post(), const int16_t* prev_mv = nullptr) {
    constexpr int SR = G::SR, TBX = G::TBX, TBY = G::TBY;
    using P = PTileGeo<G>;
    uint32_t* const b4w = reinterpret_cast<uint32_t*>(S.un);
    uint16_t* const list = reinterpret_cast<uint16_t*>(b4w + P::B4);
    constexpr int kUnDw = 2 * (VBS ? PTileGeoVbs<G>::U64 : PTileGeo<G, HALFTQ>::U64);
    int dense4 = 0;
#ifndef SO_DENSE_ONE
    if constexpr (3 * G::DCS + 32 <= kUnDw) {
        const int d = (int)((reinterpret_cast<uintptr_t>(b4w) - reinterpret_cast<uintptr_t>(S.win)) / 4);
        dense4 = d + ((8 - d) & 31);
    }
#endif
    const Sea2Lds L{S.win, b4w, S.curt, S.a4, list, S.lcount, S.keys, S.st, count_ops, dense4};
    RefSet refs{};
    refs.p[0] = ref;
#ifndef SO_PROF_PHASE
#define SO_PROF_PHASE 0
#endif
    sea2_tile<G, Pre, VBS, LISTS>(L, tile, cur, refs, 1, H, W, by0, by1, SO_PROF_PHASE == 2 ? 5 : 0, pre,
                           dense_flag, prev_mv);

    const int tid = opaque_tid();
    SO_SEA_STAMP(5, __builtin_amdgcn_s_memtime());
    const int nbx = W / 16;
    const int tiles_x = (nbx + TBX - 1) / TBX;
    const int bx0 = (tile % tiles_x) * TBX, byt0 = by0 + (tile / tiles_x) * TBY;
    for (int i = tid; i < PTileLds<G, VBS>::NU; i += G::NTHREADS) {
        SO_MARK(decode_keys);
        int32_t rec4[4];
        decode_key(S.keys[i], SR, rec4);
        S.mer[i].set(rec4);
        const int gbx = bx0 + i % TBX, gby = byt0 + i / TBX;
        if (out_best && i < G::NBLK && gbx < nbx && gby < by1) {
            int32_t* ob = out_best + ((size_t)(gby - by0) * nbx + gbx) * 4;
            ob[0] = S.mer[i][0]; ob[1] = S.mer[i][1]; ob[2] = S.mer[i][2]; ob[3] = S.mer[i][3];
        }
    }
    SO_MARK(keys_tail);
    if (fb_out != nullptr && tid == 0) store_sc1_i32(fb_out, (int)S.st[0]);
    if (tid == 0) S.fwd_flags = 0u;
    __syncthreads();
    SO_SEA_STAMP(6, __builtin_amdgcn_s_memtime());
    constexpr bool kFwdMfma = !VBS && SO_FWD_MFMA && SO_PROF_PHASE != 1;
    if constexpr (kFwdMfma) {
        const int ln = tid & 63;
        float cs[4];
#pragma unroll
        for (int s = 0; s < 4; ++s) cs[s] = dct16_f32(ln & 15, 4 * (ln >> 4) + s);
        for (int g = tid >> 6; g < G::NBLK; g += G::NW)
            fwd_mfma<G>(S, g, ln, cs, bx0, byt0, nbx, by1, qp_rd, qp_row, qp_map);
        __syncthreads();
#ifdef SO_FWD_COUNT
        if (tid == 0) S.st[2] = (uint32_t)__builtin_popcount(S.fwd_flags);
#endif
    }
    {
        const int ln = tid & 63, w = tid >> 6;
        int gq = w * G::TQ_BPW + (ln >> 4);
        bool qs = false;
        if constexpr (kFwdMfma) {
            const uint32_t m = S.fwd_flags;
            if (m != 0u && gq < G::NBLK) gq = fwd_order<G::NBLK>(m, gq);
            qs = !((m >> gq) & 1u);
        }
        if (SO_PROF_PHASE == 1 && ln < 16 * G::TQ_BPW && gq < G::NBLK) {
            const int bxl = gq % G::TBX, byl = gq / G::TBX, l = ln & 15;
            const int gbx = bx0 + bxl, gby = byt0 + byl;
            if (gbx < nbx && gby < by1) {
                const uint32_t* crow = S.curt + (byl * 16 + l) * G::CPD + bxl * 4;
                so_v4u v;
                for (int k = 0; k < 4; ++k) v[k] = crow[k];
                *reinterpret_cast<so_v4u*>(o.recon + (size_t)(gby * 16 + l) * W + gbx * 16) = v;
            }
        } else if (ln < 16 * G::TQ_BPW && gq < G::NBLK) {
            if constexpr (VBS)
                tq16_vbs_fwd<G, SC1, HALO>(S, gq, ln & 15, S.un + gq * kTqScratchVbs, bx0, byt0, nbx, by0, by1, W, qp_rd,
                                           qp_row, qp_map, lam, o);
            else
                tq16_exact<G, SC1, HALO, TOK, HALFTQ, ZSKIP>(S, gq, ln & 15, S.un + gq * (HALFTQ ? kTqScratchHalf : kTqScratch), bx0,
                                              byt0, nbx, by0, by1, W, qp_rd,
                                              qp_row, qp_map, o, hl, qs);
        }
    }
    if constexpr (VBS) {
        if (SO_PROF_PHASE != 1) {
            __syncthreads();
            const int ln = tid & 63, gq = (tid >> 6) * G::TQ_BPW + (ln >> 4);
            if (ln < 16 * G::TQ_BPW && gq < G::NBLK)
                tq16_vbs_inv<G, SC1, HALO>(S, gq, ln & 15, S.un, bx0, byt0, nbx, by0, by1, W, qp_rd,
                                           qp_row, qp_map, o, hl);
        }
    }
    SO_SEA_STAMP(7, __builtin_amdgcn_s_memtime());
    SO_MARK(post);
    post();
    if constexpr (SC1) asm volatile("s_waitcnt vmcnt(0)" ::: "memory");
    SO_SEA_STAMP(14, __builtin_amdgcn_s_memtime());
    __syncthreads();
}



template <class G>
SO_DEV void tq16_pass1(PTileLds<G>& S, int g, int l, double* scratch, int bx0, int byt0, int nbx, int by1, int qp_rd,
                       const int32_t* __restrict__ qp_row, const PFrameOut& o, int32_t* __restrict__ t1) {
    constexpr int SR = G::SR, TBX = G::TBX;
    const int bxl = g % TBX, byl = g / TBX;
    const int gbx = bx0 + bxl, gby = byt0 + byl;
    if (gbx < nbx && gby < by1) {
        const size_t b = (size_t)gby * nbx + gbx;
        const int qpr = qp_row ? qp_row[gby] : qp_rd;
        const int dx = S.mer[g][0], dy = S.mer[g][1], rf = S.mer[g][2], sad = S.mer[g][3];
        const int prow = byl * 16 + SR + dy + l, pcol = bxl * 16 + SR + dx;
        const uint32_t* crow = S.curt + (byl * 16 + l) * G::CPD + bxl * 4;
        int res[16];
        {
            uint32_t pw[4];
            win_row16<G::RP>(S.win, prow, pcol, pw);
#pragma unroll
            for (int k = 0; k < 4; ++k) {
                const uint32_t cw = crow[k];
#pragma unroll
                for (int e = 0; e < 4; ++e)
                    res[4 * k + e] = (int)((cw >> (8 * e)) & 255) - (int)((pw[k] >> (8 * e)) & 255);
            }
            const so_v4u pv{pw[0], pw[1], pw[2], pw[3]};
            uint8_t* const rp = o.recon + (size_t)(gby * 16 + l) * (nbx * 16) + gbx * 16;
            asm volatile("global_store_dwordx4 %0, %1, off sc1" ::"v"(rp), "v"(pv) : "memory");
        }
        double tcr[16];
        xform2d_rows<16, false>(scratch, l, res, tcr, SO_TQ_TW());
        constexpr double kRne = 0x1.8p52;
        int tc[16], q[16];
#pragma unroll
        for (int c = 0; c < 16; ++c) tc[c] = (int)(uint32_t)__builtin_bit_cast(uint64_t, tcr[c] + kRne);
        quant_row_int<16>(tc, l, qpr, q);
        const int tok = block_tokens<16>(nullptr, l, q);
        {
            uint32_t w[8];
#pragma unroll
            for (int k = 0; k < 8; ++k) w[k] = (uint32_t)(uint16_t)tc[2 * k] | ((uint32_t)tc[2 * k + 1] << 16);
            const so_v4u v0{w[0], w[1], w[2], w[3]}, v1{w[4], w[5], w[6], w[7]};
            int16_t* const qp_ = o.qtc + b * 256 + l * 16;
            asm volatile("global_store_dwordx4 %0, %1, off sc1" ::"v"(qp_), "v"(v0) : "memory");
            asm volatile("global_store_dwordx4 %0, %1, off offset:16 sc1" ::"v"(qp_), "v"(v1) : "memory");
        }
        if (l < 12) store_sc1_i16(o.mv + b * 12 + l, l == 0 ? dx : l == 1 ? dy : l == 2 ? rf : 0);
        if (l == 0) {
            o.split[b] = 0;
            o.mae[b] = sad;
            store_sc1_i32(t1 + b, tok);
        }
    }
}

SO_DEV void row16_any(const uint8_t* p, uint32_t (&w)[4]) {
    const uint32_t* pa = reinterpret_cast<const uint32_t*>((uintptr_t)p & ~(uintptr_t)3);
    const uint32_t sh = (uint32_t)((uintptr_t)p & 3);
    uint32_t q5[5];
#pragma unroll
    for (int k = 0; k < 5; ++k) q5[k] = pa[k];
#pragma unroll
// ... 189 lines not shown
                break;
        }
#endif
        __builtin_amdgcn_s_sleep(1);
        const uint32_t now = (uint32_t)(__builtin_amdgcn_s_memrealtime() - t0), gap = now - last;
        last = now;
        if (gap >= (uint32_t)kRunGapTicks) {
            susp += gap;
            __hip_atomic_fetch_add(&ws[kRunGapWord], one, __ATOMIC_RELAXED, __HIP_MEMORY_SCOPE_AGENT);
        }
        const uint32_t active = now - susp;
        if (!esc && active > (uint32_t)kRunEscalateTicks) {
            esc = true;
            const uint32_t v2 = (need && !sysl) ? rmw_read(c) : raw;
            const uint32_t v3 = (need && !sysl) ? __hip_atomic_load(c, __ATOMIC_RELAXED, __HIP_MEMORY_SCOPE_AGENT) : raw;
            if (__builtin_amdgcn_ballot_w64(need && !sysl && !ok && v2 == w.want && v3 != w.want) != 0)
                __hip_atomic_fetch_add(&ws[kRunStaleWord], one, __ATOMIC_RELAXED, __HIP_MEMORY_SCOPE_AGENT);
        }
        if (active > (uint32_t)w.limit) {
            __hip_atomic_fetch_add(&ws[kRunTimeoutWord], one, __ATOMIC_RELAXED, __HIP_MEMORY_SCOPE_AGENT);
            const uint32_t claim = __builtin_amdgcn_readfirstlane(
                __hip_atomic_fetch_add(&ws[kRunClaimWord], one, __ATOMIC_RELAXED, __HIP_MEMORY_SCOPE_AGENT));
            if (claim == 0u) {
                const uint32_t rv = (need && !sysl) ? rmw_read(c) : raw;
                const uint64_t bneed = __builtin_amdgcn_ballot_w64(need);
                const uint64_t bsys = __builtin_amdgcn_ballot_w64(need && sysl);
                const uint64_t brmw = __builtin_amdgcn_ballot_w64(need && !sysl && rv == w.want);
                const uint32_t other = (uint32_t)__builtin_amdgcn_ds_bpermute(((lane - 20) & 63) << 2, (int)raw);
                uint32_t hw, xcc;
                asm volatile("s_getreg_b32 %0, hwreg(HW_REG_HW_ID)" : "=s"(hw));
                asm volatile("s_getreg_b32 %0, hwreg(HW_REG_XCC_ID)" : "=s"(xcc));
                if (lane >= 20 && lane < 32)
                    __hip_atomic_store(&ws[kRunDiagWord + lane], other, __ATOMIC_RELAXED, __HIP_MEMORY_SCOPE_AGENT);
                if (lane == 0) {
                    const uint32_t rec[19] = {(uint32_t)w.task, (uint32_t)w.f, (uint32_t)w.dep, (uint32_t)w.tile, w.want,
                                              w.sys_want, (uint32_t)w.mode | (esc ? 1u << 12 : 0u), (uint32_t)bneed,
                                              (uint32_t)bsys, active, now, susp, 0u, 0xFFFFFFFFu, hw, xcc,
                                              (uint32_t)blockIdx.x, (uint32_t)gridDim.x, (uint32_t)brmw};
#pragma unroll
                    for (int i = 0; i < 19; ++i)
                        __hip_atomic_store(&ws[kRunDiagWord + 1 + i], rec[i], __ATOMIC_RELAXED, __HIP_MEMORY_SCOPE_AGENT);
                }
                const unsigned long long ta = __builtin_amdgcn_s_memrealtime();
                uint32_t arrive = 0xFFFFFFFFu;
                for (;;) {
                    const uint32_t x = sysl ? __hip_atomic_load(c, __ATOMIC_RELAXED, __HIP_MEMORY_SCOPE_SYSTEM)
                                            : (need ? rmw_read(c) : 0u);
                    const uint32_t el = (uint32_t)(__builtin_amdgcn_s_memrealtime() - ta);
                    if (__builtin_amdgcn_ballot_w64(need && x != (sysl ? w.sys_want : w.want)) == 0) {
                        arrive = el;
                        break;
                    }
                    if (el > 5000000u) break;
                    __builtin_amdgcn_s_sleep(8);
                }
                if (lane == 14)
                    __hip_atomic_store(&ws[kRunDiagWord + 14], arrive, __ATOMIC_RELAXED, __HIP_MEMORY_SCOPE_AGENT);
                if (lane == 0)
                    __hip_atomic_store(&ws[kRunDiagWord], SO_P_RUN_DIAG_MAGIC, __ATOMIC_RELAXED,
                                       __HIP_MEMORY_SCOPE_AGENT);
            }
            break;
        }
    }
    return raw;
}


SO_DEV uint32_t run_dequeue(uint32_t* ws) {
    uint32_t r;
    uint64_t sv;
    asm volatile(
        "s_mov_b64 %1, exec\n\t"
        "s_mov_b64 exec, 1\n\t"
        "global_atomic_add %0, %2, %3, off sc0\n\t"
        "s_waitcnt vmcnt(0)\n\t"
        "s_mov_b64 exec, %1"
        : "=&v"(r), "=&s"(sv)
        : "v"(ws), "v"(1u)
        : "memory");
    return r;
}

template <int NW, int MODE, bool VBS = false, bool HOOKS = false, bool UQP = false, bool ZSKIP = false>
__global__ void __launch_bounds__(NW * 64)
__attribute__((amdgpu_waves_per_eu(VBS ? SO_VBS_WPE : (NW >= 16 ? SO_PTILE_WPE16 : SO_SEA2_WPE))))
p_run_kernel(const PRunArgs a, int nframes, const uint8_t* __restrict__ ref0, int H, int W,
             int qp_rd, const int32_t* __restrict__ qp_row_arg, uint32_t* __restrict__ ws, int ws_stamp_base,
             const PRunStripe sp, double lam) {
    static_assert(!UQP || VBS, "the uniform-QP instantiation is the VBS run's");
    static_assert(!ZSKIP || (MODE == kRunSingle && !HOOKS && (!VBS || UQP)),
                  "the zero-skip / latency-lists instantiation is the one-GPU run's");
    constexpr int LISTS = VBS && MODE == kRunSingle && UQP ? (ZSKIP ? 2 : 1) : 0;
    const int32_t* __restrict__ const qp_row = UQP ? nullptr : qp_row_arg;
    using G = Sea2GeoT<NW>;
    __shared__ PTileLds<G, VBS> S;
    __shared__ int s_task;
    __shared__ int s_dense;
    const int tid = threadIdx.x;
    const int nbx = W / 16;
    constexpr bool STRIPE = MODE == kRunStripe, FPIPE = MODE == kRunFPipe || MODE == kRunFPipe2P;
    constexpr bool TWOP = MODE == kRunTwoPass || MODE == kRunFPipe2P;
    static_assert(!(VBS && (TWOP || MODE == kRunStripe)), "VBS runs: one GPU and the frame pipeline");
    static_assert(!HOOKS || MODE == kRunSingle, "test hooks: the one-GPU run only");
    const int count_ops = HOOKS ? sp.count_ops : 0;
    const int by0 = STRIPE ? sp.by0 : 0, by1 = STRIPE ? sp.by1 : H / 16;
    const int tiles_x = (nbx + G::TBX - 1) / G::TBX, ntr = (by1 - by0 + G::TBY - 1) / G::TBY;
    const int ntiles = tiles_x * ntr;
    constexpr bool MERGE2P = MODE == kRunTwoPass;
    const int lag2 = ntiles - (tiles_x + 1);
    const int per_frame = TWOP && !MERGE2P ? 2 * ntiles : ntiles;
    const int ntasks = per_frame * nframes + (MERGE2P ? lag2 : 0);
    uint32_t* const done = ws + kRunDoneBase;
    uint32_t* const tilefb = ws + kRunDoneBase + 2 * (size_t)kRunMax * ntiles + (size_t)kRunMax * nbx * (H / 16);
    const int wave = __builtin_amdgcn_readfirstlane(tid >> 6);
    const int lane = tid & 63;
    const uint32_t one = lane == 0 ? 1u : 0u;
    __shared__ uint32_t s_fbsum;
    __shared__ unsigned long long s_ops;
    if (tid == 0) {
        s_fbsum = 0;
        s_ops = 0;
    }
#ifdef SO_MARKS_COUNT
    if (tid < 64) s_mark_cnt[tid] = 0u;
#endif
    const uint32_t ep0 = __builtin_amdgcn_readfirstlane(
        __hip_atomic_load(&ws[kRunEpochWord], __ATOMIC_RELAXED, __HIP_MEMORY_SCOPE_AGENT)) + 1u;
#ifndef SO_EP_REG
    __shared__ uint32_t s_ep;
    if (tid == 0) s_ep = ep0;
#define ep ((uint32_t)__builtin_amdgcn_readfirstlane(*(lds_vu32p)&s_ep))
#else
    const uint32_t ep = ep0;
#endif
    uint32_t nxt_v = 0;
    bool nxt_taken = false;
    for (;;) {
        SO_MARK(loop_top);
        if (wave == 0) {
            if (!nxt_taken) nxt_v = run_dequeue(ws);
            s_task = (int)__builtin_amdgcn_readfirstlane(nxt_v);
            s_dense = 0;
        }
        nxt_taken = false;
        __syncthreads();
        const int task = __builtin_amdgcn_readfirstlane(s_task);
        if (task >= ntasks) break;
#ifdef SO_STAMPS
        unsigned long long* const rec = g_run_stamps ? g_run_stamps + (size_t)(ws_stamp_base + task) * 16 : nullptr;
        SO_STAMP_REC_SET(rec);
        if (tid == 0 && rec) rec[8] = __builtin_amdgcn_s_memrealtime();
#endif
        const int u2 = MERGE2P ? task - lag2 : -1;
        const bool has1 = !MERGE2P || task < nframes * ntiles;
        const int u = has1 ? task : u2;
        const int f = u / per_frame;
        int tile = u - f * per_frame, pass = has1 ? 1 : 2;
        if constexpr (TWOP && !MERGE2P) {
            const int L = sp.p2lag, k = tile, k1 = k - L * tiles_x, nb2 = (ntr - L) * 2 * tiles_x;
            if (k1 < 0) {
                tile = k;
            } else if (k1 < nb2) {
                const int j = k1 / (2 * tiles_x), rem = k1 - j * 2 * tiles_x;
                if (rem < tiles_x) {
                    tile = (j + L) * tiles_x + rem;
                } else {
                    pass = 2;
                    tile = j * tiles_x + rem - tiles_x;
                }
            } else {
                pass = 2;
                tile = (ntr - L) * tiles_x + (k1 - nb2);
            }
        }
        const int ty = tile / tiles_x, tx = tile - ty * tiles_x;
        const bool first_row = ty == 0, last_row = ty == ntr - 1;
        const int dep = (MODE == kRunSingle || MODE == kRunTwoPass) ? a.dep[f] : f - 1;
        const auto wait_ref = [&]() {
            if (wave != 0) return;
            const int gprev = (STRIPE ? sp.gbase : 0) + f - 1;
            const bool remote = STRIPE && (first_row ? sp.my_up_flags != nullptr : false);
            const bool remote_dn = STRIPE && (last_row ? sp.my_dn_flags != nullptr : false);
            if (!FPIPE && dep < 0 && !remote && !remote_dn) return;
            SO_MARK(wait_w0);
#ifdef SO_STAMPS
            if (lane == 0 && rec) rec[9] = __builtin_amdgcn_s_memrealtime();
#endif
            const int lane = opaque_tid() & 63;
            const int nx = tx + lane % 3 - 1, ny = ty + lane / 3 - 1;
            const bool need = (FPIPE || dep >= 0) && lane < 9 && nx >= 0 && nx < tiles_x && ny >= 0 && ny < ntr;
            const uint32_t* c = done + (size_t)(dep > 0 ? dep : 0) * ntiles + (need ? ny * tiles_x + nx : 0);
            bool rneed = false;
            if constexpr (FPIPE) {
                c = sp.my_dn_flags + (size_t)(sp.gbase + f) * ntiles + (need ? ny * tiles_x + nx : 0);
                rneed = need;
            }
            if constexpr (STRIPE) {
                const int rx = tx + (lane - 9) % 3 - 1;
                if (lane >= 9 && lane < 12 && remote && rx >= 0 && rx < tiles_x) {
                    c = sp.my_up_flags + (size_t)gprev * tiles_x + rx;
                    rneed = true;
                } else if (lane >= 12 && lane < 15 && remote_dn && rx >= 0 && rx < tiles_x) {
                    c = sp.my_dn_flags + (size_t)gprev * tiles_x + rx;
                    rneed = true;
                }
            }
            constexpr unsigned long long kWaitLimit = (STRIPE || FPIPE) ? 200000000ull : 5000000ull;
            const bool fbl = MODE == kRunSingle && lane == 9 && dep >= 0;
            if (fbl) c = tilefb + (size_t)dep * ntiles + tile;
#ifdef SO_RUN_PROFILE
            const unsigned long long t0 = __builtin_amdgcn_s_memrealtime();
#endif
            const RunWait rw{task, f, dep, tile, MODE | (VBS ? 16 : 0) | (pass << 8), ep, sp.epoch, kWaitLimit};
            const uint32_t raw = run_poll(c, need || rneed, (STRIPE || FPIPE) && rneed, ws, rw);
            SO_RUN_PROF(51, (__builtin_amdgcn_s_memrealtime() - t0) * 25);
#ifdef SO_STAMPS
            if (lane == 0 && rec) rec[10] = __builtin_amdgcn_s_memrealtime();
#endif
#if SO_RUN_ACQUIRE
            __builtin_amdgcn_fence(__ATOMIC_ACQUIRE, "agent");
            asm volatile("s_waitcnt vmcnt(0)" ::: "memory");
#endif
            if (MODE == kRunSingle && dep >= 0 && (f & (SO_DENSE_PROBE - 1)) != 0) {
                const uint32_t fb = (uint32_t)__builtin_amdgcn_readlane((int)raw, 9);
                if (lane == 0) s_dense = fb >= (uint32_t)SO_DENSE_THR ? 1 : 0;
            }
        };
#ifndef SO_DEQ_LATE
        const auto take_next = [&]() {
            if (wave == 0) nxt_v = run_dequeue(ws);
            nxt_taken = true;
        };
#else
        const NoPre take_next{};
#endif
        const uint8_t* ref = FPIPE ? sp.land0 + (long long)(sp.gbase + f) * sp.stride
                                   : (MODE == kRunSingle || TWOP) ? a.ref[f] : (f ? a.out[f - 1].recon : ref0);
        if constexpr (TWOP) {
            const int nb = nbx * (H / 16);
#ifdef SO_RUN_PROFILE
            const unsigned long long pt0 = __builtin_amdgcn_s_memtime();
#endif
            const auto pass1_unit = [&]() {
                int32_t* const t1 = sp.t1 + (size_t)f * nb;
                const int bx0 = tx * G::TBX, byt0 = ty * G::TBY;
                using P = PTileGeo<G>;
                uint32_t* const b4w = reinterpret_cast<uint32_t*>(S.un);
                const Sea2Lds L{S.win, b4w, S.curt, S.a4, reinterpret_cast<uint16_t*>(b4w + P::B4), S.lcount, S.keys,
                                S.st, count_ops};
                RefSet refs{};
                refs.p[0] = ref;
                sea2_tile<G>(L, tile, a.cur[f], refs, 1, H, W, 0, by1, 0, wait_ref, nullptr,
                             MODE == kRunTwoPass && dep >= 0 ? a.out[dep].mv : nullptr);
                for (int i = tid; i < G::NBLK; i += G::NTHREADS) {
                    int32_t rec4[4];
                    decode_key(S.keys[i], G::SR, rec4);
                    S.mer[i].set(rec4);
                }
                __syncthreads();
                SO_MARK(p1_tq);
                const int t2 = opaque_tid(), ln = t2 & 63, gq = (t2 >> 6) * G::TQ_BPW + (ln >> 4);
                if (ln < 16 * G::TQ_BPW && gq < G::NBLK)
                    tq16_pass1<G>(S, gq, ln & 15, S.un + gq * kTqScratch, bx0, byt0, nbx, by1, qp_rd, qp_row, a.out[f],
                                  t1);
                SO_MARK(p1_flag);
                asm volatile("s_waitcnt vmcnt(0)" ::: "memory");
                __syncthreads();
                if (wave == 0)
                    __hip_atomic_store(sp.p1done + (size_t)f * ntiles + tile, ep, __ATOMIC_RELAXED,
                                       __HIP_MEMORY_SCOPE_AGENT);
                SO_RUN_PROF(48, __builtin_amdgcn_s_memtime() - pt0);
            };
            const auto pass2_unit = [&](int f2, int tile2) {
                int32_t* const t1 = sp.t1 + (size_t)f2 * nb;
                const int ty2 = tile2 / tiles_x;
                const int bx0 = (tile2 - ty2 * tiles_x) * G::TBX, byt0 = ty2 * G::TBY;
                const uint8_t* const ref2 = FPIPE ? sp.land0 + (long long)(sp.gbase + f2) * sp.stride : a.ref[f2];
                SO_MARK(p2_wait);
                if (wave == 0) {
                    const uint32_t* c = sp.p1done + (size_t)f2 * ntiles + ty2 * tiles_x + (lane < tiles_x ? lane : 0);
                    const RunWait rw{task, f2, -2, tile2, MODE | (2 << 8), ep, sp.epoch, FPIPE ? 200000000ull : 5000000ull};
                    run_poll(c, lane < tiles_x, false, ws, rw);
                    __builtin_amdgcn_fence(__ATOMIC_ACQUIRE, "agent");
                    asm volatile("s_waitcnt vmcnt(0)" ::: "memory");
                    SO_RUN_PROF(50, __builtin_amdgcn_s_memtime() - pt0);
                }
                __syncthreads();
                SO_MARK(p2_sums);
                if (wave < G::TBY) {
                    const int row = byt0 + wave;
                    uint32_t sum = 0;
                    if (row < by1)
                        for (int bx = lane; bx < nbx; bx += 64) sum += (uint32_t)t1[(size_t)row * nbx + bx];
                    sum = wave_sum_u32(sum);
                    if (lane == 0) S.msum[wave] = (int32_t)sum;
                }
                __syncthreads();
                const int code = FPIPE ? a.dep[f2] : -1;
                uint8_t* const push = code >= 0 ? ((code & 1) ? sp.peer_up0 : sp.peer_dn0) +
                                                      (long long)(code >> 1) * sp.stride : nullptr;
                SO_MARK(p2_tq);
                const int t2 = opaque_tid(), ln = t2 & 63, gq = (t2 >> 6) * G::TQ_BPW + (ln >> 4);
                if (ln < 16 * G::TQ_BPW && gq < G::NBLK)
                    tq16_pass2<G>(S, gq, ln & 15, S.un + gq * kTqScratch, bx0, byt0, nbx, by1, W, qp_rd, qp_row, sp.roi,
                                  sp.qp_lo, sp.qp_hi, a.cur[f2], ref2, a.out[f2], t1, push);
                SO_MARK(p2_flag);
                asm volatile("s_waitcnt vmcnt(0)" ::: "memory");
                __syncthreads();
// ... 37 lines not shown
            }
        } else if constexpr (STRIPE) {
            const int gf = sp.gbase + f;
            PHalo hl{};
            if (first_row && sp.peer_up0) {
                hl.up = sp.peer_up0 + (long long)gf * sp.stride;
                hl.up_end = by0 * 16 + 16;
            }
            if (last_row && sp.peer_dn0) {
                hl.dn = sp.peer_dn0 + (long long)gf * sp.stride;
                hl.dn_begin = by1 * 16 - 16;
            }
            ptile_body<G, true, decltype(wait_ref), true, false, false, decltype(take_next)>(
                S, tile, a.cur[f], ref, H, W, by0, by1, qp_rd, qp_row, nullptr, nullptr, a.out[f], wait_ref, hl, 0.0,
                nullptr, nullptr, count_ops, take_next, f > 0 ? a.out[f - 1].mv : nullptr);
            if (wave == 0) {
                __hip_atomic_store(done + (size_t)f * ntiles + tile, ep, __ATOMIC_RELAXED,
                                       __HIP_MEMORY_SCOPE_AGENT);
                if (lane == 0 && hl.up)
                    __hip_atomic_store(sp.peer_up_flags + (size_t)gf * tiles_x + tx, sp.epoch, __ATOMIC_RELAXED,
                                       __HIP_MEMORY_SCOPE_SYSTEM);
                if (lane == 1 && hl.dn)
                    __hip_atomic_store(sp.peer_dn_flags + (size_t)gf * tiles_x + tx, sp.epoch, __ATOMIC_RELAXED,
                                       __HIP_MEMORY_SCOPE_SYSTEM);
            }
        } else {
#ifdef SO_RUN_PROFILE
            const unsigned long long pt0 = __builtin_amdgcn_s_memtime();
#endif
            ptile_body<G, true, decltype(wait_ref), false, false, VBS, decltype(take_next), false, ZSKIP && !VBS, LISTS>(
                S, tile, a.cur[f], ref, H, W, 0, by1, qp_rd, qp_row, nullptr, nullptr, a.out[f], wait_ref, PHalo{}, lam,
                &s_dense, reinterpret_cast<int32_t*>(tilefb) + (size_t)f * ntiles + tile, count_ops, take_next,
                !VBS && dep >= 0 ? a.out[dep].mv : nullptr);
            SO_RUN_PROF(52, __builtin_amdgcn_s_memtime() - pt0);
            SO_MARK(done_flag);
            if (wave == 0 && !(HOOKS && task + 1 == sp.lose_task))
                __hip_atomic_store(done + (size_t)f * ntiles + tile, ep, __ATOMIC_RELAXED,
                                       __HIP_MEMORY_SCOPE_AGENT);
        }
        SO_MARK(task_end);
        if (pass == 1 && tid == 0) {
            s_fbsum += S.st[0];
            if constexpr (HOOKS) s_ops += S.st[2];
        }
#ifdef SO_STAMPS
        if (tid == 0 && rec) {
            uint32_t hw, xcc;
            asm volatile("s_getreg_b32 %0, hwreg(HW_REG_HW_ID)" : "=s"(hw));
            asm volatile("s_getreg_b32 %0, hwreg(HW_REG_XCC_ID)" : "=s"(xcc));
            rec[11] = __builtin_amdgcn_s_memrealtime();
            rec[12] = ((unsigned long long)xcc << 32) | hw;
            rec[13] = __builtin_amdgcn_s_memtime();
        }
#endif
    }
#ifdef SO_MARKS_COUNT
    __syncthreads();
    if (tid < kMarkCount && g_mark_counts) atomicAdd(&g_mark_counts[tid], s_mark_cnt[tid]);
#endif
    if (wave == 0) {
        const uint32_t fbsum = __builtin_amdgcn_readfirstlane(s_fbsum);
        if (fbsum != 0u)
            __hip_atomic_fetch_add(&ws[kRunFallbackWord], lane == 0 ? fbsum : 0u, __ATOMIC_RELAXED,
                                   __HIP_MEMORY_SCOPE_AGENT);
        const unsigned long long ops = s_ops;
        if (ops != 0ull)
            __hip_atomic_fetch_add(reinterpret_cast<unsigned long long*>(ws + kRunSadOpsWord), lane == 0 ? ops : 0ull,
                                   __ATOMIC_RELAXED, __HIP_MEMORY_SCOPE_AGENT);
    }
    if (wave == 0) {
        const uint32_t o = __builtin_amdgcn_readfirstlane(
            __hip_atomic_fetch_add(&ws[kRunExitWord], one, __ATOMIC_RELAXED, __HIP_MEMORY_SCOPE_AGENT));
        if (o == gridDim.x - 1) {
            __hip_atomic_store(&ws[0], 0u, __ATOMIC_RELAXED, __HIP_MEMORY_SCOPE_AGENT);
            __hip_atomic_store(&ws[kRunExitWord], 0u, __ATOMIC_RELAXED, __HIP_MEMORY_SCOPE_AGENT);
            __hip_atomic_store(&ws[kRunEpochWord], ep, __ATOMIC_RELAXED, __HIP_MEMORY_SCOPE_AGENT);
        }
    }
}
#ifndef SO_EP_REG
#undef ep
#endif

static size_t run_tiles(int H, int W, int tbx, int tby) {
    return (size_t)((W / 16 + tbx - 1) / tbx) * ((H / 16 + tby - 1) / tby);
}
size_t p_run_workspace_words(int H, int W) {
    using G = Sea2Geo;
    return (size_t)kRunDoneBase + 3 * (size_t)kRunMax * run_tiles(H, W, G::TBX, G::TBY) +
           (size_t)kRunMax * (W / 16) * (H / 16);
}

constexpr size_t kLdsPerCuObserved = 161280;
static_assert(sizeof(PTileLds<Sea2GeoT<SO_PTILE_NW>, true>) + 64 <= kLdsPerCuObserved / 3,
              "the VBS run's LDS no longer fits three workgroups per gfx950 CU");
static int run_shape(const void* kernel, int* ncu, int* per_cu) {
    static std::mutex mu;
    static std::map<std::pair<int, const void*>, std::pair<int, int>> cache;
    int dev = 0;
    const hipError_t e = hipGetDevice(&dev);
    if (e != hipSuccess) {
        set_error("p_run: hipGetDevice: %s", hipGetErrorString(e));
        return (int)e;
    }
    std::lock_guard<std::mutex> lk(mu);
    const auto key = std::make_pair(dev, kernel);
    auto it = cache.find(key);
    if (it == cache.end()) {
        int n = 0, p = 0;
        if (hipDeviceGetAttribute(&n, hipDeviceAttributeMultiprocessorCount, dev) != hipSuccess || n <= 0) n = 256;
        if (hipOccupancyMaxActiveBlocksPerMultiprocessor(&p, kernel, SO_PTILE_NW * 64, 0) != hipSuccess || p <= 0) p = 1;
        hipDeviceProp_t prop{};
        const bool gfx950 = hipGetDeviceProperties(&prop, dev) == hipSuccess &&
                            std::strncmp(prop.gcnArchName, "gfx950", 6) == 0;
        hipFuncAttributes fa{};
        if (gfx950 && hipFuncGetAttributes(&fa, kernel) == hipSuccess && fa.sharedSizeBytes > 0) {
            const size_t g = (fa.sharedSizeBytes + 511) & ~(size_t)511;
            const int by_lds = (int)(kLdsPerCuObserved / g);
            if (by_lds >= 1 && by_lds < p) p = by_lds;
        }
        it = cache.emplace(key, std::make_pair(n, p)).first;
    }
    *ncu = it->second.first;
    *per_cu = it->second.second;
    return SO_OK;
}

int p_run_capacity(int vbs, int mode) {
    constexpr int NW = SO_PTILE_NW;
    const void* ks[13];
    int n = 0;
    const auto add = [&](int m, const void* k) {
        if (mode < 0 || mode == m) ks[n++] = k;
    };
    if (vbs) {
        add(kRunSingle, reinterpret_cast<const void*>(p_run_kernel<NW, kRunSingle, true>));
        add(kRunSingle, reinterpret_cast<const void*>(p_run_kernel<NW, kRunSingle, true, true>));
        add(kRunSingle, reinterpret_cast<const void*>(p_run_kernel<NW, kRunSingle, true, false, true>));
        add(kRunSingle, reinterpret_cast<const void*>(p_run_kernel<NW, kRunSingle, true, true, true>));
        add(kRunSingle, reinterpret_cast<const void*>(p_run_kernel<NW, kRunSingle, true, false, true, true>));
        add(kRunFPipe, reinterpret_cast<const void*>(p_run_kernel<NW, kRunFPipe, true>));
        add(kRunFPipe, reinterpret_cast<const void*>(p_run_kernel<NW, kRunFPipe, true, false, true>));
    } else {
        add(kRunSingle, reinterpret_cast<const void*>(p_run_kernel<NW, kRunSingle, false>));
        add(kRunSingle, reinterpret_cast<const void*>(p_run_kernel<NW, kRunSingle, false, true>));
        add(kRunSingle, reinterpret_cast<const void*>(p_run_kernel<NW, kRunSingle, false, false, false, true>));
        add(kRunStripe, reinterpret_cast<const void*>(p_run_kernel<NW, kRunStripe, false>));
        add(kRunFPipe, reinterpret_cast<const void*>(p_run_kernel<NW, kRunFPipe, false>));
        add(kRunTwoPass, reinterpret_cast<const void*>(p_run_kernel<NW, kRunTwoPass, false>));
        add(kRunFPipe2P, reinterpret_cast<const void*>(p_run_kernel<NW, kRunFPipe2P, false>));
    }
    if (n == 0) return -SO_E_INVALID;
    int best = 0;
    for (int i = 0; i < n; ++i) {
        int ncu = 0, per_cu = 0;
        const int rc = run_shape(ks[i], &ncu, &per_cu);
        if (rc != SO_OK) return -rc;
        if (i == 0 || ncu * per_cu < best) best = ncu * per_cu;
    }
    return best;
}

template <int MODE, bool VBS = false>
static int p_run_launch_t(const uint8_t* const* curs, int nframes, const uint8_t* ref0, int H, int W, int qp_rd,
                          const int32_t* qp_row, const PFrameOut* outs, uint32_t* ws, const PRunStripe& sp0,
                          int max_wg, hipStream_t st, const uint8_t* const* refs = nullptr,
                          const int* deps = nullptr, int conc = 1, double lam = 0.0) {
    using G = Sea2GeoT<SO_PTILE_NW>;
    const bool hook_set = option(SO_OPT_COUNT_SAD_OPS) != 0 || option(SO_OPT_TEST_LOSE_FLAG) != 0;
    if (hook_set && MODE != kRunSingle) {
        set_error("p_run: SO_OPT_COUNT_SAD_OPS / SO_OPT_TEST_LOSE_FLAG apply to the one-GPU run only (so_encode_p_run, "
                  "so_encode_p_runs); this run kind has no hook instantiation");
        return SO_E_INVALID;
    }
    const bool hooks = MODE == kRunSingle && hook_set;
    const bool uqp = VBS && qp_row == nullptr;
    constexpr bool ZS_OK = MODE == kRunSingle && !VBS;
    const bool zskip = ZS_OK && !hooks && option(SO_OPT_RUN_ZERO_SKIP) != 0;
    constexpr bool VL_OK = MODE == kRunSingle && VBS;
    const bool vlat_ok = VL_OK && uqp && !hooks && SO_VBS_BALLOT_LATENCY;
    const void* const kfn =
        hooks ? (uqp ? reinterpret_cast<const void*>(p_run_kernel<SO_PTILE_NW, MODE, VBS, MODE == kRunSingle, VBS>)
                     : reinterpret_cast<const void*>(p_run_kernel<SO_PTILE_NW, MODE, VBS, MODE == kRunSingle>))
              : (uqp     ? reinterpret_cast<const void*>(p_run_kernel<SO_PTILE_NW, MODE, VBS, false, VBS>)
                 : zskip ? reinterpret_cast<const void*>(p_run_kernel<SO_PTILE_NW, MODE, VBS, false, false, ZS_OK>)
                         : reinterpret_cast<const void*>(p_run_kernel<SO_PTILE_NW, MODE, VBS, false>));
    if (hooks && option(SO_OPT_TEST_LOSE_FLAG) != 0) {
        hipStreamCaptureStatus cs = hipStreamCaptureStatusNone;
        if (hipStreamIsCapturing(st, &cs) != hipSuccess || cs != hipStreamCaptureStatusNone) {
            set_error("p_run: SO_OPT_TEST_LOSE_FLAG is set while the stream is capturing (the graph would lose a "
                      "flag on every replay)");
            return SO_E_INVALID;
        }
    }
    int ncu = 0, per_cu = 0;
    {
        const int rc = run_shape(kfn, &ncu, &per_cu);
        if (rc != SO_OK) return rc;
    }
    const int nbx = W / 16;
    const int rows = MODE == kRunStripe ? sp0.by1 - sp0.by0 : H / 16;
    const long ntiles = (long)((nbx + G::TBX - 1) / G::TBX) * ((rows + G::TBY - 1) / G::TBY);
    for (int f0 = 0; f0 < nframes; f0 += kRunMax) {
        const int n = nframes - f0 < kRunMax ? nframes - f0 : kRunMax;
        PRunArgs a{};
        for (int i = 0; i < n; ++i) {
            const int g = f0 + i;
            const int d = deps ? deps[g] : g - 1;
            a.cur[i] = curs[g];
            a.out[i] = outs[g];
            if (MODE == kRunFPipe || MODE == kRunFPipe2P) {
                a.ref[i] = nullptr;
                a.dep[i] = deps ? deps[g] : -1;
                continue;
            }
            a.ref[i] = d >= 0 ? outs[d].recon : (refs ? refs[g] : ref0);
            a.dep[i] = d >= f0 ? d - f0 : -1;
        }
        int pcu = (int)((ntiles * conc + ncu - 1) / ncu);
        if (pcu > per_cu) pcu = per_cu;
#ifdef SO_AB
        if (const char* e = getenv("SO_RUN_PER_CU")) {
            const int v = atoi(e);
            if (v > 0 && v <= per_cu) pcu = v;
        }
#endif
        long grid = (long)ncu * pcu;
        if (grid > ntiles * n) grid = ntiles * n;
        if (max_wg > 0 && grid > max_wg) grid = max_wg;
        PRunStripe sp = sp0;
        sp.gbase = sp0.gbase + f0;
        sp.count_ops = option(SO_OPT_COUNT_SAD_OPS);
        sp.lose_task = f0 == 0 ? option(SO_OPT_TEST_LOSE_FLAG) : 0;
        if (MODE == kRunTwoPass || MODE == kRunFPipe2P) {
            const int tiles_x = (nbx + G::TBX - 1) / G::TBX, ntr = (rows + G::TBY - 1) / G::TBY;
            int lag = (int)((grid + tiles_x - 1) / tiles_x);
            if (sp0.p2lag > 0 && sp0.p2lag < lag) lag = sp0.p2lag;
#ifdef SO_AB
            if (const char* e = getenv("SO_P2LAG")) lag = atoi(e);
#endif
            sp.p2lag = lag < 1 ? 1 : (lag > ntr ? ntr : lag);
        }
        const uint8_t* const r0 = f0 ? outs[f0 - 1].recon : ref0;
#define SO_P_RUN_GO(HK, UQ, ZS)                                                                                         \
    hipLaunchKernelGGL((p_run_kernel<SO_PTILE_NW, MODE, VBS, HK, UQ, ZS>), dim3((unsigned)grid), dim3(SO_PTILE_NW * 64), \
                       0, st, a, n, r0, H, W, qp_rd, qp_row, ws, (int)(f0 * ntiles), sp, lam)
        if (hooks && uqp)
            SO_P_RUN_GO(MODE == kRunSingle, VBS, false);
        else if (hooks)
            SO_P_RUN_GO(MODE == kRunSingle, false, false);
        else if (uqp && vlat_ok && ntiles < grid)
            SO_P_RUN_GO(false, VBS, VL_OK);
        else if (uqp)
            SO_P_RUN_GO(false, VBS, false);
        else if (zskip)
            SO_P_RUN_GO(false, false, ZS_OK);
        else
            SO_P_RUN_GO(false, false, false);
#undef SO_P_RUN_GO
        const int rc = check_launch("p_run_kernel");
        if (rc != SO_OK) return rc;
    }
    return SO_OK;
}

int p_run_launch(const uint8_t* const* curs, int nframes, const uint8_t* ref0, int H, int W, int qp_rd,
                 const int32_t* qp_row, int vbs, double lam, const PFrameOut* outs, uint32_t* ws, hipStream_t st) {
    PRunStripe sp{};
    sp.by0 = 0;
    sp.by1 = H / 16;
    if (vbs)
        return p_run_launch_t<kRunSingle, true>(curs, nframes, ref0, H, W, qp_rd, qp_row, outs, ws, sp, 0, st, nullptr,
                                                nullptr, 1, lam);
    return p_run_launch_t<kRunSingle>(curs, nframes, ref0, H, W, qp_rd, qp_row, outs, ws, sp, 0, st);
}

int p_runs_launch(const uint8_t* const* curs, int nframes, const uint8_t* const* refs, const int* deps, int conc,
                  int H, int W, int qp_rd, const int32_t* qp_row, int vbs, double lam, const PFrameOut* outs,
                  uint32_t* ws, hipStream_t st) {
    PRunStripe sp{};
    sp.by0 = 0;
    sp.by1 = H / 16;
    if (vbs)
        return p_run_launch_t<kRunSingle, true>(curs, nframes, nullptr, H, W, qp_rd, qp_row, outs, ws, sp, 0, st, refs,
                                                deps, conc, lam);
    return p_run_launch_t<kRunSingle>(curs, nframes, nullptr, H, W, qp_rd, qp_row, outs, ws, sp, 0, st, refs, deps,
                                           conc);
}

int32_t* p_run_t1_region(uint32_t* ws, int H, int W) {
    return reinterpret_cast<int32_t*>(ws + kRunDoneBase + 2 * (size_t)kRunMax * run_tiles(H, W, Sea2Geo::TBX, Sea2Geo::TBY));
}

bool p_run_2pass_fused_ok(int H, int W) {
    const int tiles_x = (W / 16 + Sea2Geo::TBX - 1) / Sea2Geo::TBX;
    return 2 * tiles_x < run_tiles(H, W, Sea2Geo::TBX, Sea2Geo::TBY);
}

int p_run_2pass_launch(const uint8_t* const* curs, int nframes, const uint8_t* ref0, int H, int W, int qp_rd,
                       const int32_t* qp_row, const int32_t* roi, int qp_lo, int qp_hi, const PFrameOut* outs,
                       uint32_t* ws, hipStream_t st) {
    if (!p_run_2pass_fused_ok(H, W)) {
        set_error("so_encode_p_run_2pass (fused): needs three tile rows (H > %d)", 2 * 16 * Sea2Geo::TBY);
        return SO_E_UNSUPPORTED;
    }
    PRunStripe sp{};
    sp.by0 = 0;
    sp.by1 = H / 16;
    sp.p1done = ws + kRunDoneBase + (size_t)kRunMax * run_tiles(H, W, Sea2Geo::TBX, Sea2Geo::TBY);
    sp.t1 = reinterpret_cast<int32_t*>(sp.p1done + (size_t)kRunMax * run_tiles(H, W, Sea2Geo::TBX, Sea2Geo::TBY));
    sp.roi = roi;
    sp.qp_lo = qp_lo;
    sp.qp_hi = qp_hi;
    return p_run_launch_t<kRunTwoPass>(curs, nframes, ref0, H, W, qp_rd, qp_row, outs, ws, sp, 0, st, nullptr,
                                            nullptr, 2);
}

int p_run_stripe_launch(const uint8_t* const* curs, int nframes, const uint8_t* ref0, int H, int W, int qp_rd,
                        const int32_t* qp_row, const PFrameOut* outs, uint32_t* ws, const PRunStripe& sp, int max_wg,
                        hipStream_t st) {
    return p_run_launch_t<kRunStripe>(curs, nframes, ref0, H, W, qp_rd, qp_row, outs, ws, sp, max_wg, st);
}

int p_run_fpipe_launch(const uint8_t* const* curs, int nframes, int H, int W, int qp_rd, const int32_t* qp_row,
                       int vbs, double lam, const PFrameOut* outs, uint32_t* ws, const PRunStripe& sp, int max_wg,
                       hipStream_t st, const int* push) {
    if (vbs)
        return p_run_launch_t<kRunFPipe, true>(curs, nframes, nullptr, H, W, qp_rd, qp_row, outs, ws, sp, max_wg, st,
                                               nullptr, push, 1, lam);
    return p_run_launch_t<kRunFPipe>(curs, nframes, nullptr, H, W, qp_rd, qp_row, outs, ws, sp, max_wg, st,
                                          nullptr, push);
}

int p_run_fpipe_2pass_launch(const uint8_t* const* curs, int nframes, int H, int W, int qp_rd, const int32_t* qp_row,
                             const PFrameOut* outs, uint32_t* ws, const PRunStripe& sp0, int max_wg, hipStream_t st,
                             const int* push) {
    PRunStripe sp = sp0;
    sp.p1done = ws + kRunDoneBase + (size_t)kRunMax * run_tiles(H, W, Sea2Geo::TBX, Sea2Geo::TBY);
// ... 179 lines not shown
```

### streamoptima_amd/csrc/so_run.h

```cpp
#pragma once
#include "so_common.h"

namespace so {

constexpr int kRunMax = 32;

struct PFrameOut {
    uint8_t* split;
    int16_t* mv;
    int16_t* qtc;
    int32_t* tokens;
    int32_t* mae;
    uint8_t* recon;
    int32_t* sse;
    int32_t* qpmap;
};

struct PRunStripe {
    int by0, by1;
    uint8_t* peer_up0;
    uint8_t* peer_dn0;
    long long stride;
    const uint32_t* my_up_flags;
    const uint32_t* my_dn_flags;
    uint32_t* peer_up_flags;
    uint32_t* peer_dn_flags;
    uint32_t epoch;
    int gbase;
    const uint8_t* land0;
    uint32_t* p1done;
    int32_t* t1;
    const int32_t* roi;
    int qp_lo, qp_hi;
    int p2lag;
    int count_ops;
    int lose_task;
};

size_t p_run_workspace_words(int H, int W);
int p_run_capacity(int vbs, int mode = -1);
bool p_run_2pass_fused_ok(int H, int W);
int32_t* p_run_t1_region(uint32_t* ws, int H, int W);
int p_run_launch(const uint8_t* const* curs, int nframes, const uint8_t* ref0, int H, int W, int qp_rd,
                 const int32_t* qp_row, int vbs, double lam, const PFrameOut* outs, uint32_t* ws, hipStream_t st);
int p_runs_launch(const uint8_t* const* curs, int nframes, const uint8_t* const* refs, const int* deps, int conc,
                  int H, int W, int qp_rd, const int32_t* qp_row, int vbs, double lam, const PFrameOut* outs,
                  uint32_t* ws, hipStream_t st);
int p_run_2pass_launch(const uint8_t* const* curs, int nframes, const uint8_t* ref0, int H, int W, int qp_rd,
                       const int32_t* qp_row, const int32_t* roi, int qp_lo, int qp_hi, const PFrameOut* outs,
                       uint32_t* ws, hipStream_t st);
int p_run_stripe_launch(const uint8_t* const* curs, int nframes, const uint8_t* ref0, int H, int W, int qp_rd,
                        const int32_t* qp_row, const PFrameOut* outs, uint32_t* ws, const PRunStripe& sp, int max_wg,
                        hipStream_t st);
int p_run_fpipe_launch(const uint8_t* const* curs, int nframes, int H, int W, int qp_rd, const int32_t* qp_row,
                       int vbs, double lam, const PFrameOut* outs, uint32_t* ws, const PRunStripe& sp, int max_wg,
                       hipStream_t st, const int* push);
int p_run_fpipe_2pass_launch(const uint8_t* const* curs, int nframes, int H, int W, int qp_rd, const int32_t* qp_row,
                             const PFrameOut* outs, uint32_t* ws, const PRunStripe& sp, int max_wg, hipStream_t st,
                             const int* push);

}
```

Baseline: 162,300.

## Add tall three-row tiles for one-GPU P-run with LDS-lean split-double transform

Adds a taller tile geometry (three block rows instead of two) for the plain single-GPU P-run kernel. Each tile now covers more blocks, so search-window staging is amortised over more of them and the halo overhead drops. To keep three workgroups per CU in LDS, the transform uses a new 32-bit-lane transpose that moves doubles as two halves, and MVs and current pixels are re-read from LDS to ease register pressure. An auto heuristic picks tall tiles only when there are enough tiles to fill the device, and falls back to a separate short-tile kernel otherwise. The cost is extra LDS round trips in the transform and fewer tiles, which can mean worse load balance.

```diff
diff --git a/include/streamoptima.h b/include/streamoptima.h
--- a/include/streamoptima.h
+++ b/include/streamoptima.h
@@ -48,6 +48,7 @@
 #define SO_OPT_COUNT_SAD_OPS 5
 #define SO_OPT_TEST_LOSE_FLAG 6
 #define SO_OPT_RUN_ZERO_SKIP 7
+#define SO_OPT_RUN_TALL_TILES 8
 int so_set_option(int option, int value);
 int so_get_option(int option);
 
@@ -61,6 +62,7 @@
 size_t so_p_run_workspace_elems(int H, int W);
 int so_p_run_resident_workgroups(int vbs);
 int so_p_run_mode_resident_workgroups(int mode, int vbs);
+int so_p_run_tile_rows(int H, int W, int conc);
 int so_encode_p_run(const uint8_t* const* curs, int nframes, const uint8_t* ref0, int H, int W,
                     int bs, int sr, int qp_rd, const int32_t* qp_row, int vbs, double lam,
                     uint8_t* const* out_split,
diff --git a/streamoptima_amd/_lib.py b/streamoptima_amd/_lib.py
--- a/streamoptima_amd/_lib.py
+++ b/streamoptima_amd/_lib.py
@@ -36,6 +36,7 @@
     "so_p_run_resident_workgroups": ([_i], _i),
     "so_p_run_mode_resident_workgroups": ([_i, _i], _i),
     "so_p_run_2pass_fused": ([_i, _i], _i),
+    "so_p_run_tile_rows": ([_i, _i, _i], _i),
     "so_encode_p_run": ([_vp, _i, _vp, _i, _i, _i, _i, _i, _vp, _i, _d, _vp, _vp, _vp, _vp, _vp, _vp, _vp, _vp, _vp],
                         _i),
     "so_encode_p_run_2pass": ([_vp, _i, _vp, _i, _i, _i, _i, _i, _vp, _vp, _i, _i, _vp, _vp, _vp, _vp, _vp, _vp, _vp,
@@ -95,6 +96,7 @@
 TOKENS_ONLY = 2
 OPT_RUN_2PASS_FUSED, OPT_FASTME_SERIAL, OPT_FASTME_SEGMENT, OPT_FASTME_WARMUP, OPT_COUNT_SAD_OPS = 1, 2, 3, 4, 5
 OPT_RUN_ZERO_SKIP = 7
+OPT_RUN_TALL_TILES = 8
 OPT_TEST_LOSE_FLAG = 6
 
 EXPORTED = tuple(_SIGS)
diff --git a/streamoptima_amd/csrc/so_block.h b/streamoptima_amd/csrc/so_block.h
--- a/streamoptima_amd/csrc/so_block.h
+++ b/streamoptima_amd/csrc/so_block.h
@@ -160,6 +160,43 @@
     wave_sync();
 #pragma unroll
     for (int c = 0; c < N; ++c) v[c] = lds[l * P + c];
+    if constexpr (INVERSE) dct::dct3<N>(v, tw); else dct::dct2<N>(v, tw);
+#pragma unroll
+    for (int c = 0; c < N; ++c) out_row[c] = v[c];
+    wave_sync();
+}
+
+template <bool INVERSE, class TWt>
+SO_DEV void xform2d_rows_dw(double* lds, int l, const int* in_row, double* out_row, const TWt& tw) {
+    constexpr int N = 16, P = N + 1;
+    typedef __attribute__((address_space(3))) uint32_t* lds_u32p;
+    lds_u32p rowp = (lds_u32p)(reinterpret_cast<uint32_t*>(lds) + l * P);
+    lds_u32p colp = (lds_u32p)(reinterpret_cast<uint32_t*>(lds) + l);
+    asm volatile("" : "+v"(rowp), "+v"(colp));
+    double v[N];
+    {
+#pragma unroll
+        for (int c = 0; c < N; ++c) rowp[c] = (uint32_t)in_row[c];
+        wave_sync();
+        int x[N];
+#pragma unroll
+        for (int r = 0; r < N; ++r) x[r] = (int)colp[r * P];
+        wave_sync();
+        if constexpr (INVERSE) dct::dct3_16_i(x, v, tw); else dct::dct2_16_i(x, v, tw);
+    }
+    uint32_t lo[N];
+#pragma unroll
+    for (int r = 0; r < N; ++r) colp[r * P] = (uint32_t)__builtin_bit_cast(uint64_t, v[r]);
+    wave_sync();
+#pragma unroll
+    for (int c = 0; c < N; ++c) lo[c] = rowp[c];
+    wave_sync();
+#pragma unroll
+    for (int r = 0; r < N; ++r) colp[r * P] = (uint32_t)(__builtin_bit_cast(uint64_t, v[r]) >> 32);
+    wave_sync();
+#pragma unroll
+    for (int c = 0; c < N; ++c)
+        v[c] = __builtin_bit_cast(double, ((uint64_t)rowp[c] << 32) | (uint64_t)lo[c]);
     if constexpr (INVERSE) dct::dct3<N>(v, tw); else dct::dct2<N>(v, tw);
 #pragma unroll
     for (int c = 0; c < N; ++c) out_row[c] = v[c];
diff --git a/streamoptima_amd/csrc/so_capi.hip b/streamoptima_amd/csrc/so_capi.hip
--- a/streamoptima_amd/csrc/so_capi.hip
+++ b/streamoptima_amd/csrc/so_capi.hip
@@ -22,10 +22,13 @@
     va_end(ap);
 }
 
-static std::atomic<int> g_opt[8] = {0, 1, 0, 32, 32, 0, 0, 0};
+#ifndef SO_RUN_TALL_DEFAULT
+#define SO_RUN_TALL_DEFAULT -1
+#endif
+static std::atomic<int> g_opt[9] = {0, 1, 0, 32, 32, 0, 0, 0, SO_RUN_TALL_DEFAULT};
 
 int option(int id) {
-    return (id > 0 && id < 8) ? g_opt[id].load(std::memory_order_relaxed) : 0;
+    return (id > 0 && id < 9) ? g_opt[id].load(std::memory_order_relaxed) : 0;
 }
 
 int me_launch(const uint8_t* cur, const RefSet& refs, int nref, int H, int W, int bs, int sr, int by0, int by1,
@@ -302,6 +305,7 @@
     const bool ok = (opt == SO_OPT_RUN_2PASS_FUSED || opt == SO_OPT_FASTME_SERIAL || opt == SO_OPT_COUNT_SAD_OPS ||
                      opt == SO_OPT_RUN_ZERO_SKIP)
                         ? (value == 0 || value == 1)
+                    : opt == SO_OPT_RUN_TALL_TILES                               ? (value >= -1 && value <= 1)
                     : opt == SO_OPT_FASTME_SEGMENT                               ? value >= 1
                     : opt == SO_OPT_FASTME_WARMUP || opt == SO_OPT_TEST_LOSE_FLAG ? value >= 0
                                                                                  : false;
@@ -408,6 +412,19 @@
     const int n = p_run_capacity(vbs ? 1 : 0);
     if (n <= 0) {
         set_error("so_p_run_resident_workgroups: device query failed");
+        return SO_E_INVALID;
+    }
+    return n;
+}
+
+int so_p_run_tile_rows(int H, int W, int conc) {
+    if (H < 16 || W < 128 || H % 16 != 0 || W % 128 != 0 || conc < 1) {
+        set_error("so_p_run_tile_rows: H %d W %d conc %d (H a multiple of 16, W of 128, conc >= 1)", H, W, conc);
+        return SO_E_INVALID;
+    }
+    const int n = p_run_tile_rows(H, W, conc);
+    if (n <= 0) {
+        set_error("so_p_run_tile_rows: device query failed");
         return SO_E_INVALID;
     }
     return n;
diff --git a/streamoptima_amd/csrc/so_me.hip b/streamoptima_amd/csrc/so_me.hip
--- a/streamoptima_amd/csrc/so_me.hip
+++ b/streamoptima_amd/csrc/so_me.hip
@@ -4,6 +4,7 @@
 #include <cstring>
 #include <map>
 #include <mutex>
+#include <type_traits>
 #include <utility>
 
 #include "so_block.h"
@@ -499,16 +500,17 @@
 #ifndef SO_PTILE_WPE16
 #define SO_PTILE_WPE16 8
 #endif
-template <int NW_, int TPX_ = 128>
+template <int NW_, int TPX_ = 128, int TBY_ = 2, bool TQDW_ = false>
 struct Sea2GeoT {
     static constexpr int SR = 16, NT = 17;
-    static constexpr int TPX = TPX_, TBX = TPX / 16, TPY = 32, TBY = 2;
+    static constexpr int TPX = TPX_, TBX = TPX / 16, TBY = TBY_, TPY = 16 * TBY;
+    static constexpr bool TQDW = TQDW_;
     static constexpr int WR = TPY + 2 * SR;
     static constexpr int WD = (TPX + 2 * SR) / 4;
     static constexpr int RP = WD + 1;
     static constexpr int B4R = WR - 3, B4C = TPX + 2 * SR - 3, B4P = 4 * RP;
     static constexpr int TQ_BPW = TPX == 128 ? 4 : 2;
-    static constexpr int B4BAND = NW_ >= 16 ? 3 : 6;
+    static constexpr int B4BAND = TBY_ == 3 ? 7 : (NW_ >= 16 ? 3 : 6);
     static constexpr int B4NB = (B4R + B4BAND - 1) / B4BAND;
     static constexpr int B4RS = B4NB * B4BAND;
     static constexpr int NBLK = TBX * TBY;
@@ -1001,20 +1003,24 @@
     SO_MARK(stage_cur);
     for (int i = tid; i < G::NBLK * (VBS ? 5 : 1); i += G::NTHREADS) keys[i] = kNoKey;
     constexpr int WTPR = G::NTHREADS / G::WR, WNPT = (RP + WTPR - 1) / WTPR;
-    static_assert(G::NTHREADS % G::WR == 0, "window staging");
+    constexpr bool WALL = WTPR * G::WR == G::NTHREADS;
+    static_assert(WTPR >= 1 && WTPR * WNPT >= RP, "window staging");
     const int wwr = tid / WTPR, wc0 = tid - wwr * WTPR;
     const bool win_int = x0 - SR >= 0 && x0 - SR + 4 * RP <= W && y0 - SR >= 0 && y0 - SR + G::WR <= H;
     if (x0 + CP <= W && y0 + G::TPY <= H) {
-        constexpr int TPR = G::NTHREADS / G::TPY, NPT = (CP / 4) / TPR;
-        static_assert(G::NTHREADS % G::TPY == 0 && (CP / 4) % TPR == 0, "current-tile staging");
+        constexpr int TPR = G::NTHREADS / G::TPY, NPT = (CP / 4 + TPR - 1) / TPR;
+        constexpr bool CALL = G::NTHREADS % G::TPY == 0 && (CP / 4) % TPR == 0;
+        static_assert(TPR >= 1 && TPR <= CP / 4, "current-tile staging");
         SO_MARK(stage_cur_int);
         const int rr = tid / TPR, c0 = tid - rr * TPR;
         const uint32_t* src = reinterpret_cast<const uint32_t*>(cur + (size_t)(y0 + rr) * W + x0) + c0;
         uint32_t v[NPT];
 #pragma unroll
-        for (int k = 0; k < NPT; ++k) v[k] = src[k * TPR];
-#pragma unroll
-        for (int k = 0; k < NPT; ++k) curt[rr * G::CPD + c0 + k * TPR] = v[k];
+        for (int k = 0; k < NPT; ++k)
+            if (CALL || (rr < G::TPY && c0 + k * TPR < CP / 4)) v[k] = src[k * TPR];
+#pragma unroll
+        for (int k = 0; k < NPT; ++k)
+            if (CALL || (rr < G::TPY && c0 + k * TPR < CP / 4)) curt[rr * G::CPD + c0 + k * TPR] = v[k];
     } else {
         SO_MARK(stage_cur_edge);
         constexpr int N = G::TPY * CP / 4, IT = (N + G::NTHREADS - 1) / G::NTHREADS;
@@ -1069,10 +1075,10 @@
             const uint32_t* src = reinterpret_cast<const uint32_t*>(ref + (size_t)(y0 - SR + wwr) * W + (x0 - SR)) + wc0;
 #pragma unroll
             for (int k = 0; k < WNPT; ++k)
-                if (wc0 + k * WTPR < RP) wv0[k] = src[k * WTPR];
+                if ((WALL || wwr < G::WR) && wc0 + k * WTPR < RP) wv0[k] = src[k * WTPR];
 #pragma unroll
             for (int k = 0; k < WNPT; ++k)
-                if (wc0 + k * WTPR < RP) win[wwr * RP + wc0 + k * WTPR] = wv0[k];
+                if ((WALL || wwr < G::WR) && wc0 + k * WTPR < RP) win[wwr * RP + wc0 + k * WTPR] = wv0[k];
         } else {
             SO_MARK(stage_win_edge);
             constexpr int N = G::WR * RP, IT = (N + G::NTHREADS - 1) / G::NTHREADS;
@@ -1447,6 +1453,11 @@
 #define SO_PTILE_TOK_HALF 1
 #endif
 constexpr int kTqScratchHalf = 16 * 9;
+constexpr int kTqScratchDw = 16 * 17 / 2;
+template <class G, bool HALFTQ>
+constexpr int tq_scratch() {
+    return HALFTQ ? kTqScratchHalf : (G::TQDW ? kTqScratchDw : kTqScratch);
+}
 #ifndef SO_FWD_MFMA
 #define SO_FWD_MFMA 0
 #endif
@@ -1454,7 +1465,7 @@
 struct PTileGeo {
     static constexpr int B4 = (G::B4RS * G::B4P + 4) / 4;
     static constexpr int LIST = G::NW * G::CAPL / 2;
-    static constexpr int TQD = G::NBLK * (HALFTQ ? kTqScratchHalf : kTqScratch);
+    static constexpr int TQD = G::NBLK * tq_scratch<G, HALFTQ>();
     static constexpr int U64 = ((B4 + LIST + 1) / 2 > TQD) ? (B4 + LIST + 1) / 2 : TQD;
 };
 constexpr int kTqScratchVbs = 288;
@@ -1563,6 +1574,8 @@
             static_assert(!HALFTQ || TOK, "the half scratch carries the forward transform only");
             if constexpr (HALFTQ)
                 xform2d_fwd_i_half(dl, l, res, tcr, SO_TQ_TW());
+            else if constexpr (G::TQDW)
+                xform2d_rows_dw<false>(dl, l, res, tcr, SO_TQ_TW());
             else
                 xform2d_rows<16, false>(dl, l, res, tcr, SO_TQ_TW());
             SO_MARK(tq_quant);
@@ -1604,9 +1617,15 @@
             SO_MARK(tq_sse_records);
             int e2 = 0;
             if (o.sse) {
+                const uint32_t* crow2 = crow;
+                if constexpr (G::TQDW) {
+                    int g2 = g, l2 = l;
+                    asm volatile("" : "+v"(g2), "+v"(l2));
+                    crow2 = S.curt + ((g2 / TBX) * 16 + l2) * G::CPD + (g2 % TBX) * 4;
+                }
 #pragma unroll
                 for (int k = 0; k < 4; ++k) {
-                    const uint32_t cw = crow[k];
+                    const uint32_t cw = crow2[k];
 #pragma unroll
                     for (int e = 0; e < 4; ++e) {
                         const int d = (int)((cw >> (8 * e)) & 255) - (rec[4 * k + e] & 255);
@@ -1622,7 +1641,10 @@
             double rd[16];
             dequant_row_int<16>(q, l, qpr, dq);
             SO_MARK(tq_inv);
-            xform2d_rows<16, true>(dl, l, dq, rd, SO_TQ_TW());
+            if constexpr (G::TQDW)
+                xform2d_rows_dw<true>(dl, l, dq, rd, SO_TQ_TW());
+            else
+                xform2d_rows<16, true>(dl, l, dq, rd, SO_TQ_TW());
             SO_MARK(tq_recon);
             int rec[16];
             {
@@ -1650,11 +1672,22 @@
         } else {
             sse = full();
         }
-        if (l < 12) o.mv[b * 12 + l] = (int16_t)(l == 0 ? dx : l == 1 ? dy : l == 2 ? rf : 0);
+        int mdx = dx, mdy = dy, mrf = rf, msad = sad;
+        if constexpr (G::TQDW) {
+            int g2 = g;
+            asm volatile("" : "+v"(g2));
+            lds_vu32p mp = (lds_vu32p)reinterpret_cast<const uint32_t*>(&S.mer[g2]);
+            const uint32_t w0 = mp[0], w1 = mp[1];
+            mdx = (int)(int16_t)(w0 & 0xFFFFu);
+            mdy = (int)w0 >> 16;
+            mrf = (int)(int16_t)(w1 & 0xFFFFu);
+            msad = (w1 >> 16) == 0xFFFFu ? -1 : (int)(w1 >> 16);
+        }
+        if (l < 12) o.mv[b * 12 + l] = (int16_t)(l == 0 ? mdx : l == 1 ? mdy : l == 2 ? mrf : 0);
         if (l == 0) {
             o.split[b] = 0;
             o.tokens[b] = tok;
-            o.mae[b] = sad;
+            o.mae[b] = msad;
             if (o.sse) o.sse[b] = sse;
         }
     }
@@ -2157,7 +2190,7 @@
                 tq16_vbs_fwd<G, SC1, HALO>(S, gq, ln & 15, S.un + gq * kTqScratchVbs, bx0, byt0, nbx, by0, by1, W, qp_rd,
                                            qp_row, qp_map, lam, o);
             else
-                tq16_exact<G, SC1, HALO, TOK, HALFTQ, ZSKIP>(S, gq, ln & 15, S.un + gq * (HALFTQ ? kTqScratchHalf : kTqScratch), bx0,
+                tq16_exact<G, SC1, HALO, TOK, HALFTQ, ZSKIP>(S, gq, ln & 15, S.un + gq * tq_scratch<G, HALFTQ>(), bx0,
                                               byt0, nbx, by0, by1, W, qp_rd,
                                               qp_row, qp_map, o, hl, qs);
         }
@@ -2513,18 +2546,24 @@
     return r;
 }
 
-template <int NW, int MODE, bool VBS = false, bool HOOKS = false, bool UQP = false, bool ZSKIP = false>
-__global__ void __launch_bounds__(NW * 64)
-__attribute__((amdgpu_waves_per_eu(VBS ? SO_VBS_WPE : (NW >= 16 ? SO_PTILE_WPE16 : SO_SEA2_WPE))))
-p_run_kernel(const PRunArgs a, int nframes, const uint8_t* __restrict__ ref0, int H, int W,
-             int qp_rd, const int32_t* __restrict__ qp_row_arg, uint32_t* __restrict__ ws, int ws_stamp_base,
-             const PRunStripe sp, double lam) {
+#ifndef SO_RUN_SHORT_TQDW
+#define SO_RUN_SHORT_TQDW 0
+#endif
+template <int NW>
+using RunGeoTall = Sea2GeoT<NW, 128, 3, true>;
+template <int NW>
+using RunGeoShort = Sea2GeoT<NW, 128, 2, SO_RUN_SHORT_TQDW != 0>;
+template <int MODE, bool VBS, bool HOOKS, bool UQP>
+constexpr bool kRunHasTall = MODE == kRunSingle && !VBS && !HOOKS && !UQP;
+template <class G, int MODE, bool VBS, bool HOOKS, bool UQP, bool ZSKIP>
+SO_DEV void p_run_body(const PRunArgs& a, int nframes, const uint8_t* __restrict__ ref0, int H, int W,
+                       int qp_rd, const int32_t* __restrict__ qp_row_arg, uint32_t* __restrict__ ws, int ws_stamp_base,
+                       const PRunStripe& sp, double lam) {
     static_assert(!UQP || VBS, "the uniform-QP instantiation is the VBS run's");
     static_assert(!ZSKIP || (MODE == kRunSingle && !HOOKS && (!VBS || UQP)),
                   "the zero-skip / latency-lists instantiation is the one-GPU run's");
     constexpr int LISTS = VBS && MODE == kRunSingle && UQP ? (ZSKIP ? 2 : 1) : 0;
     const int32_t* __restrict__ const qp_row = UQP ? nullptr : qp_row_arg;
-    using G = Sea2GeoT<NW>;
     __shared__ PTileLds<G, VBS> S;
     __shared__ int s_task;
     __shared__ int s_dense;
@@ -2655,7 +2694,7 @@
 #endif
             if (MODE == kRunSingle && dep >= 0 && (f & (SO_DENSE_PROBE - 1)) != 0) {
                 const uint32_t fb = (uint32_t)__builtin_amdgcn_readlane((int)raw, 9);
-                if (lane == 0) s_dense = fb >= (uint32_t)SO_DENSE_THR ? 1 : 0;
+                if (lane == 0) s_dense = fb >= (uint32_t)(SO_DENSE_THR * G::NBLK / 16) ? 1 : 0;
             }
         };
 #ifndef SO_DEQ_LATE
@@ -2859,6 +2898,27 @@
 #undef ep
 #endif
 
+#define SO_RUN_KERNEL_ATTRS(NW, VBS) \
+    __launch_bounds__(NW * 64)       \
+    __attribute__((amdgpu_waves_per_eu(VBS ? SO_VBS_WPE : (NW >= 16 ? SO_PTILE_WPE16 : SO_SEA2_WPE))))
+template <int NW, int MODE, bool VBS = false, bool HOOKS = false, bool UQP = false, bool ZSKIP = false>
+__global__ void SO_RUN_KERNEL_ATTRS(NW, VBS)
+p_run_kernel(const PRunArgs a, int nframes, const uint8_t* __restrict__ ref0, int H, int W,
+             int qp_rd, const int32_t* __restrict__ qp_row_arg, uint32_t* __restrict__ ws, int ws_stamp_base,
+             const PRunStripe sp, double lam) {
+    using G = std::conditional_t<kRunHasTall<MODE, VBS, HOOKS, UQP>, RunGeoTall<NW>, Sea2GeoT<NW>>;
+    p_run_body<G, MODE, VBS, HOOKS, UQP, ZSKIP>(a, nframes, ref0, H, W, qp_rd, qp_row_arg, ws, ws_stamp_base, sp, lam);
+}
+template <int NW, bool ZSKIP>
+__global__ void SO_RUN_KERNEL_ATTRS(NW, false)
+p_run_short_kernel(const PRunArgs a, int nframes, const uint8_t* __restrict__ ref0, int H, int W,
+                   int qp_rd, const int32_t* __restrict__ qp_row_arg, uint32_t* __restrict__ ws, int ws_stamp_base,
+                   const PRunStripe sp, double lam) {
+    p_run_body<RunGeoShort<NW>, kRunSingle, false, false, false, ZSKIP>(a, nframes, ref0, H, W, qp_rd, qp_row_arg, ws,
+                                                                         ws_stamp_base, sp, lam);
+}
+#undef SO_RUN_KERNEL_ATTRS
+
 static size_t run_tiles(int H, int W, int tbx, int tby) {
     return (size_t)((W / 16 + tbx - 1) / tbx) * ((H / 16 + tby - 1) / tby);
 }
@@ -2871,6 +2931,8 @@
 constexpr size_t kLdsPerCuObserved = 161280;
 static_assert(sizeof(PTileLds<Sea2GeoT<SO_PTILE_NW>, true>) + 64 <= kLdsPerCuObserved / 3,
               "the VBS run's LDS no longer fits three workgroups per gfx950 CU");
+static_assert(sizeof(PTileLds<RunGeoTall<SO_PTILE_NW>>) + 64 <= kLdsPerCuObserved / 3,
+              "the tall plain run's LDS no longer fits three workgroups per gfx950 CU");
 static int run_shape(const void* kernel, int* ncu, int* per_cu) {
     static std::mutex mu;
     static std::map<std::pair<int, const void*>, std::pair<int, int>> cache;
@@ -2905,7 +2967,7 @@
 
 int p_run_capacity(int vbs, int mode) {
     constexpr int NW = SO_PTILE_NW;
-    const void* ks[13];
+    const void* ks[16];
     int n = 0;
     const auto add = [&](int m, const void* k) {
         if (mode < 0 || mode == m) ks[n++] = k;
@@ -2922,6 +2984,8 @@
         add(kRunSingle, reinterpret_cast<const void*>(p_run_kernel<NW, kRunSingle, false>));
         add(kRunSingle, reinterpret_cast<const void*>(p_run_kernel<NW, kRunSingle, false, true>));
         add(kRunSingle, reinterpret_cast<const void*>(p_run_kernel<NW, kRunSingle, false, false, false, true>));
+        add(kRunSingle, reinterpret_cast<const void*>(p_run_short_kernel<NW, false>));
+        add(kRunSingle, reinterpret_cast<const void*>(p_run_short_kernel<NW, true>));
         add(kRunStripe, reinterpret_cast<const void*>(p_run_kernel<NW, kRunStripe, false>));
         add(kRunFPipe, reinterpret_cast<const void*>(p_run_kernel<NW, kRunFPipe, false>));
         add(kRunTwoPass, reinterpret_cast<const void*>(p_run_kernel<NW, kRunTwoPass, false>));
@@ -2938,12 +3002,34 @@
     return best;
 }
 
+static int p_run_tall_choice(int H, int W, int conc, bool zskip, bool* tall) {
+    const int opt = option(SO_OPT_RUN_TALL_TILES);
+    if (opt >= 0) {
+        *tall = opt != 0;
+        return SO_OK;
+    }
+    constexpr int NW = SO_PTILE_NW;
+    int ncu = 0, per_cu = 0;
+    const int rc = run_shape(zskip ? reinterpret_cast<const void*>(p_run_kernel<NW, kRunSingle, false, false, false, true>)
+                                   : reinterpret_cast<const void*>(p_run_kernel<NW, kRunSingle, false>),
+                             &ncu, &per_cu);
+    if (rc != SO_OK) return rc;
+    using GT = RunGeoTall<NW>;
+    *tall = (long long)run_tiles(H, W, GT::TBX, GT::TBY) * conc >= (long long)ncu * per_cu;
+    return SO_OK;
+}
+int p_run_tile_rows(int H, int W, int conc) {
+    bool tall = false;
+    if (p_run_tall_choice(H, W, conc, false, &tall) != SO_OK) return -1;
+    return tall ? RunGeoTall<SO_PTILE_NW>::TBY : Sea2Geo::TBY;
+}
+
 template <int MODE, bool VBS = false>
 static int p_run_launch_t(const uint8_t* const* curs, int nframes, const uint8_t* ref0, int H, int W, int qp_rd,
                           const int32_t* qp_row, const PFrameOut* outs, uint32_t* ws, const PRunStripe& sp0,
                           int max_wg, hipStream_t st, const uint8_t* const* refs = nullptr,
                           const int* deps = nullptr, int conc = 1, double lam = 0.0) {
-    using G = Sea2GeoT<SO_PTILE_NW>;
+    using GS = Sea2GeoT<SO_PTILE_NW>;
     const bool hook_set = option(SO_OPT_COUNT_SAD_OPS) != 0 || option(SO_OPT_TEST_LOSE_FLAG) != 0;
     if (hook_set && MODE != kRunSingle) {
         set_error("p_run: SO_OPT_COUNT_SAD_OPS / SO_OPT_TEST_LOSE_FLAG apply to the one-GPU run only (so_encode_p_run, "
@@ -2956,7 +3042,17 @@
     const bool zskip = ZS_OK && !hooks && option(SO_OPT_RUN_ZERO_SKIP) != 0;
     constexpr bool VL_OK = MODE == kRunSingle && VBS;
     const bool vlat_ok = VL_OK && uqp && !hooks && SO_VBS_BALLOT_LATENCY;
+    constexpr bool TALL_OK = MODE == kRunSingle && !VBS;
+    bool tall = false;
+    if (TALL_OK && !hooks) {
+        const int rc = p_run_tall_choice(H, W, conc, zskip, &tall);
+        if (rc != SO_OK) return rc;
+    }
+    const int tby = tall ? RunGeoTall<SO_PTILE_NW>::TBY : GS::TBY;
     const void* const kfn =
+        TALL_OK && !hooks && !tall
+            ? (zskip ? reinterpret_cast<const void*>(p_run_short_kernel<SO_PTILE_NW, true>)
+                     : reinterpret_cast<const void*>(p_run_short_kernel<SO_PTILE_NW, false>)) :
         hooks ? (uqp ? reinterpret_cast<const void*>(p_run_kernel<SO_PTILE_NW, MODE, VBS, MODE == kRunSingle, VBS>)
                      : reinterpret_cast<const void*>(p_run_kernel<SO_PTILE_NW, MODE, VBS, MODE == kRunSingle>))
               : (uqp     ? reinterpret_cast<const void*>(p_run_kernel<SO_PTILE_NW, MODE, VBS, false, VBS>)
@@ -2977,7 +3073,7 @@
     }
     const int nbx = W / 16;
     const int rows = MODE == kRunStripe ? sp0.by1 - sp0.by0 : H / 16;
-    const long ntiles = (long)((nbx + G::TBX - 1) / G::TBX) * ((rows + G::TBY - 1) / G::TBY);
+    const long ntiles = (long)((nbx + GS::TBX - 1) / GS::TBX) * ((rows + tby - 1) / tby);
     for (int f0 = 0; f0 < nframes; f0 += kRunMax) {
         const int n = nframes - f0 < kRunMax ? nframes - f0 : kRunMax;
         PRunArgs a{};
@@ -3010,7 +3106,7 @@
         sp.count_ops = option(SO_OPT_COUNT_SAD_OPS);
         sp.lose_task = f0 == 0 ? option(SO_OPT_TEST_LOSE_FLAG) : 0;
         if (MODE == kRunTwoPass || MODE == kRunFPipe2P) {
-            const int tiles_x = (nbx + G::TBX - 1) / G::TBX, ntr = (rows + G::TBY - 1) / G::TBY;
+            const int tiles_x = (nbx + GS::TBX - 1) / GS::TBX, ntr = (rows + GS::TBY - 1) / GS::TBY;
             int lag = (int)((grid + tiles_x - 1) / tiles_x);
             if (sp0.p2lag > 0 && sp0.p2lag < lag) lag = sp0.p2lag;
 #ifdef SO_AB
@@ -3030,7 +3126,18 @@
             SO_P_RUN_GO(false, VBS, VL_OK);
         else if (uqp)
             SO_P_RUN_GO(false, VBS, false);
-        else if (zskip)
+        else if (TALL_OK && !tall) {
+            if constexpr (TALL_OK) {
+                if (zskip)
+                    hipLaunchKernelGGL((p_run_short_kernel<SO_PTILE_NW, true>), dim3((unsigned)grid),
+                                       dim3(SO_PTILE_NW * 64), 0, st, a, n, r0, H, W, qp_rd, qp_row, ws,
+                                       (int)(f0 * ntiles), sp, lam);
+                else
+                    hipLaunchKernelGGL((p_run_short_kernel<SO_PTILE_NW, false>), dim3((unsigned)grid),
+                                       dim3(SO_PTILE_NW * 64), 0, st, a, n, r0, H, W, qp_rd, qp_row, ws,
+                                       (int)(f0 * ntiles), sp, lam);
+            }
+        } else if (zskip)
             SO_P_RUN_GO(false, false, ZS_OK);
         else
             SO_P_RUN_GO(false, false, false);
diff --git a/streamoptima_amd/csrc/so_run.h b/streamoptima_amd/csrc/so_run.h
--- a/streamoptima_amd/csrc/so_run.h
+++ b/streamoptima_amd/csrc/so_run.h
@@ -39,6 +39,7 @@
 
 size_t p_run_workspace_words(int H, int W);
 int p_run_capacity(int vbs, int mode = -1);
+int p_run_tile_rows(int H, int W, int conc);
 bool p_run_2pass_fused_ok(int H, int W);
 int32_t* p_run_t1_region(uint32_t* ws, int H, int W);
 int p_run_launch(const uint8_t* const* curs, int nframes, const uint8_t* ref0, int H, int W, int qp_rd,
```

Result: faster. 170,500 (median of 6 runs) (+5.1%).
